# toposware/certificate-stark

Hardware: AMD Instinct MI355X
Metric: proofs/sec, state_transition AIR @ 2^20 steps (complete prove(): trace gen, LDE, Blake3 commitments, constraint evaluation, composition, DEEP, FRI, 96 queries) (higher is better)
Workload: dtype u64 (63-bit prime field, Montgomery) + u32 (Blake3)

## Files before the change

certificate-stark_amd/csrc/capi.hip:

```cpp
#include <hip/hip_runtime.h>
#include <stdio.h>
#include <stdlib.h>
#include <string.h>
#include <deque>
#include <new>
#include <vector>
#include "../../include/cstark.h"
#include "air_tx_host.h"
#include "blake3.h"
#include "ctx.h"
#include "constraints.h"
#include "deep.h"
#include "ext.h"
#include "hostfield.h"
#include "ntt.h"
#include "trace_gen.h"

namespace cs { thread_local char g_err[512] = ""; }
using cs::fail;
using cs::NttPlan;
using cs::CosetTable;
using cs::PeriodicTable;
using cs::g_err;

namespace {

struct DevGuard {
    std::vector<void *> ptrs;
    bool armed = true;
    template <class T> hipError_t alloc(T **p, size_t bytes) {
        const hipError_t e = hipMalloc((void **)p, bytes);
        if (e == hipSuccess) ptrs.push_back(*p);
        return e;
    }
    void release() { armed = false; }
    ~DevGuard() { if (armed) for (void *q : ptrs) (void)hipFree(q); }
};

int get_plan(cstark_ctx *c, unsigned log_n, const NttPlan **out) {
    for (const NttPlan &p : c->plans)
        if (p.log_n == log_n) { *out = &p; return CSTARK_OK; }
    const size_t n = (size_t)1 << log_n;
    NttPlan p{log_n, nullptr, nullptr, 0};
    DevGuard g;
    HIP_TRY(g.alloc(&p.w, n * 8));
    HIP_TRY(g.alloc(&p.winv, n * 8));
    const uint64_t w = cs::host::root_of_unity(log_n);
    HIP_TRY(cs::ntt_power_table(p.w, n, w, c->stream));
    HIP_TRY(cs::ntt_power_table(p.winv, n, cs::host::inv(w), c->stream));
    p.n_inv = cs::host::inv(cs::host::from_u64(n));
    cs::NttThreeStepShape shape;
    if (cs::ntt_three_step_shape(log_n, &shape)) {
        const size_t words = cs::ntt_aux_plan_words(shape);
        HIP_TRY(g.alloc(&p.aux_w, words * 8));
        HIP_TRY(g.alloc(&p.aux_winv, words * 8));
        HIP_TRY(cs::ntt_build_aux_plan(p.aux_w, p.w, shape, c->stream));
        HIP_TRY(cs::ntt_build_aux_plan(p.aux_winv, p.winv, shape, c->stream));
    }
    c->plans.push_back(p);
    g.release();
    *out = &c->plans.back();
    return CSTARK_OK;
}

int get_coset_table(cstark_ctx *c, unsigned log_n, unsigned log_b, uint64_t offset, const CosetTable **out) {
    for (const CosetTable &t : c->cosets)
        if (t.log_n == log_n && t.log_b == log_b && t.offset == offset) { *out = &t; return CSTARK_OK; }
    const size_t n = (size_t)1 << log_n, b = (size_t)1 << log_b;
    CosetTable t{log_n, log_b, offset, nullptr};
    DevGuard g;
    HIP_TRY(g.alloc(&t.s, b * n * 8));
    const uint64_t wbn = cs::host::root_of_unity(log_n + log_b);
    uint64_t shift = offset;
    for (size_t k = 0; k < b; k++) {
        HIP_TRY(cs::ntt_power_table(t.s + k * n, n, shift, c->stream));
        shift = cs::host::mul(shift, wbn);
    }
    cs::NttThreeStepShape shape;
    if (cs::ntt_three_step_shape(log_n, &shape)) {
        const NttPlan *p;
        RC_TRY(get_plan(c, log_n, &p));
        t.aux_words = cs::ntt_aux_coset_words(shape);
        HIP_TRY(g.alloc(&t.aux, b * t.aux_words * 8));
        for (size_t k = 0; k < b; k++) HIP_TRY(cs::ntt_build_aux_coset(t.aux + k * t.aux_words, p->w, t.s + k * n, shape, c->stream));
    }
    c->cosets.push_back(t);
    g.release();
    *out = &c->cosets.back();
    return CSTARK_OK;
}

int ensure_ws(cstark_ctx *c, size_t bytes) {
    if (bytes <= c->ws_bytes) return CSTARK_OK;
    if (c->ws) { HIP_TRY(hipStreamSynchronize(c->stream)); HIP_TRY(hipFree(c->ws)); c->ws = nullptr; c->ws_bytes = 0; }
    HIP_TRY(hipMalloc(&c->ws, bytes));
    c->ws_bytes = bytes;
// ... 181 lines not shown
int get_periodic(cstark_ctx *c, unsigned depth, unsigned log_n, unsigned log_b, const PeriodicTable **out) {
    for (const PeriodicTable &t : c->periodic)
        if (t.depth == depth && t.log_n == log_n && t.log_b == log_b) { *out = &t; return CSTARK_OK; }
    if (log_n < 10) return fail(CSTARK_ERR_INVALID_ARG, "the trace must hold at least one 1024-row transaction");
    std::vector<uint64_t> cols;
    if (!cs::host::tx_periodic_columns(depth, cols)) return fail(CSTARK_ERR_INVALID_ARG, "unsupported Merkle depth");
    static_assert(cs::host::TX_CYCLE == 1 << 10, "the cycle of TransactionAir's periodic columns");
    const size_t n = (size_t)1 << log_n, b = (size_t)1 << log_b;
    PeriodicTable t{depth, log_n, log_b, nullptr, nullptr, nullptr};
    DevGuard keep;
    RC_TRY(extend_periodic_columns(c, cols, cs::host::TX_NUM_PERIODIC, 10, log_n, log_b, keep, &t.tab));
    HIP_TRY(keep.alloc(&t.coset, b * cs::CE_COSET_CONSTS * 8));
    const uint64_t g = cs::host::lde_offset();
    std::vector<uint64_t> cc(b * cs::CE_COSET_CONSTS);
    const uint64_t wbn = cs::host::root_of_unity(log_n + log_b);
    uint64_t shift = g;
    for (size_t k = 0; k < b; k++) {
        uint64_t *o = cc.data() + k * cs::CE_COSET_CONSTS;
        o[0] = shift;
        o[1] = cs::host::inv(cs::host::sub(cs::host::pow(shift, n), cs::host::ONE));
        for (int gi = 0; gi < 5; gi++) o[2 + gi] = cs::host::pow(shift, cs::host::tx_group_adjustment(gi, n, n * b));
        o[7] = cs::host::pow(shift, cs::host::tx_boundary_adjustment(n, n * b));
        o[8] = cs::host::pow(shift, n - 1);
        o[9] = 0;
        shift = cs::host::mul(shift, wbn);
    }
    HIP_TRY(hipMemcpyAsync(t.coset, cc.data(), cc.size() * 8, hipMemcpyHostToDevice, c->stream));
    const NttPlan *plan;
    RC_TRY(get_plan(c, log_n, &plan));
    HIP_TRY(keep.alloc(&t.binv, b * 2 * n * 8));
    HIP_TRY(cs::build_boundary_inverses(t.binv, plan->w, t.coset, cs::host::inv(cs::host::root_of_unity(log_n)), log_n, log_b, c->stream));
    HIP_TRY(hipStreamSynchronize(c->stream));
    keep.release();
    c->periodic.push_back(t);
    *out = &c->periodic.back();
    return CSTARK_OK;
}

int get_small_periodic(cstark_ctx *c, int air, unsigned depth, unsigned log_n, unsigned log_b, const PeriodicTable **out) {
    for (const PeriodicTable &t : c->small_periodic)
        if (t.air == air && t.depth == depth && t.log_n == log_n && t.log_b == log_b) { *out = &t; return CSTARK_OK; }
    PeriodicTable t{depth, log_n, log_b, nullptr, nullptr, nullptr, air};
    std::vector<uint64_t> cols;
    DevGuard keep;
    if (air == CSTARK_AIR_MERKLE_UPDATE) {
        if (!cs::host::merkle_periodic_columns(depth, cols)) return fail(CSTARK_ERR_INVALID_ARG, "unsupported Merkle depth");
        RC_TRY(extend_periodic_columns(c, cols, 33, 9, log_n, log_b, keep, &t.tab));
    } else if (air == CSTARK_AIR_SCHNORR) {
        cs::host::schnorr_mask_columns(cols);
        RC_TRY(extend_periodic_columns(c, cols, 36, 9, log_n, log_b, keep, &t.tab));
    } else if (air == CSTARK_AIR_RESCUE_CHAIN) {
        using namespace cs::host;
        rescue_chain_periodic_columns(cols);
        const size_t n = (size_t)1 << log_n, b = (size_t)1 << log_b;
        for (int cidx = 0; cidx < 29; cidx++) intt_small(cols.data() + (size_t)cidx * 8, 3);
        std::vector<uint64_t> tab(b * 29 * 8);
        const uint64_t wbn = root_of_unity(log_n + log_b), w8 = root_of_unity(3);
        uint64_t shift = lde_offset();
        for (size_t k = 0; k < b; k++) {
            uint64_t x = pow(shift, n / 8);
            for (int m = 0; m < 8; m++) {
                for (int cidx = 0; cidx < 29; cidx++) {
                    const uint64_t *co = cols.data() + (size_t)cidx * 8;
                    uint64_t v = 0;
                    for (int d = 7; d >= 0; d--) v = add(mul(v, x), co[d]);
                    tab[(k * 29 + cidx) * 8 + m] = v;
                }
                x = mul(x, w8);
            }
            shift = mul(shift, wbn);
        }
        HIP_TRY(keep.alloc(&t.tab, tab.size() * 8));
        HIP_TRY(hipMemcpyAsync(t.tab, tab.data(), tab.size() * 8, hipMemcpyHostToDevice, c->stream));
        HIP_TRY(hipStreamSynchronize(c->stream));
    } else {
        return fail(CSTARK_ERR_UNSUPPORTED, "AIR not available through the generic entry points");
    }
    keep.release();
    c->small_periodic.push_back(t);
    *out = &c->small_periodic.back();
    return CSTARK_OK;
}

int ce_params(cstark_ctx *c, const uint64_t *d_lde, uint64_t *d_out, uint32_t merkle_depth, uint32_t log_n, uint32_t log_blowup, uint32_t k0,
              uint32_t nk, cs::CeParams *p) {
    if (!c || !d_lde || !d_out) return fail(CSTARK_ERR_INVALID_ARG, "constraint evaluation: null argument");
    if (((uintptr_t)d_lde & 15) != 0) return fail(CSTARK_ERR_INVALID_ARG, "constraint evaluation: d_lde must be 16-byte aligned (16-byte LDS-DMA pieces)");
    if (log_n < 10 || log_n > cs::NTT_MAX_LOG_N) return fail(CSTARK_ERR_INVALID_ARG, "trace length must be 2^10 .. 2^24");
    if (log_blowup != 3) return fail(CSTARK_ERR_UNSUPPORTED, "TransactionAir needs a constraint-evaluation blowup of 8 (max degree 7, src/air.rs:76-108)");
    if ((uint64_t)k0 + nk > (1ull << log_blowup) || nk == 0) return fail(CSTARK_ERR_INVALID_ARG, "coset range exceeds the blowup factor");
    HIP_TRY(hipSetDevice(c->device));
    const PeriodicTable *pt;
    const NttPlan *plan;
    RC_TRY(get_periodic(c, merkle_depth, log_n, log_blowup, &pt));
    RC_TRY(get_plan(c, log_n, &plan));
    const uint64_t n = 1ull << log_n, ce = n << log_blowup;
    *p = cs::CeParams{};
    p->lde = d_lde; p->ptab = pt->tab; p->w = plan->w; p->coset = pt->coset; p->binv = pt->binv; p->out = d_out;
    p->w_last = cs::host::inv(cs::host::root_of_unity(log_n));
    for (int g = 0; g < 5; g++) p->adj_mod_n[g] = (uint32_t)(cs::host::tx_group_adjustment(g, n, ce) & (n - 1));
    p->badj_mod_n = (uint32_t)(cs::host::tx_boundary_adjustment(n, ce) & (n - 1));
    p->log_n = log_n; p->log_b = log_blowup; p->k0 = k0;
    return CSTARK_OK;
}

}

int tx_witness_reserve(cstark_ctx *c, size_t n, size_t d, size_t *sz, size_t *off) {
    cs::witness_segments(n, d, sz, off);
    const size_t total = off[cs::WIT_NUM_SEGMENTS];
    if (total > c->wit_bytes) {
        if (c->wit_buf) { HIP_TRY(hipStreamSynchronize(c->stream)); HIP_TRY(hipFree(c->wit_buf)); c->wit_buf = nullptr; c->wit_bytes = 0; }
        HIP_TRY(hipMalloc(&c->wit_buf, total));
        c->wit_bytes = total;
    }
    return CSTARK_OK;
}
void tx_witness_bind(cstark_ctx *c, size_t n, size_t d, const size_t *off) {
    char *base = (char *)c->wit_buf;
    cs::TxWitnessDev &dv = c->wit;
    dv.n_tx = (uint32_t)n;
    dv.depth = (uint32_t)d;
    dv.initial_roots = (const uint64_t *)(base + off[cs::WIT_INITIAL_ROOTS]);
    dv.s_old = (const uint64_t *)(base + off[cs::WIT_S_OLD]);
    dv.r_old = (const uint64_t *)(base + off[cs::WIT_R_OLD]);
    dv.s_idx = (const uint64_t *)(base + off[cs::WIT_S_IDX]);
    dv.r_idx = (const uint64_t *)(base + off[cs::WIT_R_IDX]);
    dv.s_paths = (const uint64_t *)(base + off[cs::WIT_S_PATHS]);
    dv.r_paths = (const uint64_t *)(base + off[cs::WIT_R_PATHS]);
    dv.deltas = (const uint64_t *)(base + off[cs::WIT_DELTAS]);
    dv.sig_rx = (const uint64_t *)(base + off[cs::WIT_SIG_RX]);
    dv.h_limbs = (uint64_t *)(base + off[cs::WIT_H_LIMBS]);
    dv.sig_s = (const uint8_t *)(base + off[cs::WIT_SIG_S]);
    dv.msg_tail = nullptr;
}

extern "C" {

const char *cstark_last_error(void) { return g_err; }
const char *cstark_version(void) { return "certificate-stark_amd 0.2 (gfx950)"; }

int cstark_ctx_create(int device, void *stream, cstark_ctx **out) {
    if (!out) return fail(CSTARK_ERR_INVALID_ARG, "cstark_ctx_create: out is null");
    int count = 0;
    if (hipGetDeviceCount(&count) != hipSuccess || count == 0)
        return fail(CSTARK_ERR_NO_DEVICE, "no HIP device visible (this backend has no CPU fallback)");
    if (device < 0) HIP_TRY(hipGetDevice(&device));
    if (device >= count) return fail(CSTARK_ERR_INVALID_ARG, "device index out of range");
    HIP_TRY(hipSetDevice(device));
    cstark_ctx *c = new (std::nothrow) cstark_ctx();
    if (!c) return fail(CSTARK_ERR_OOM, "host allocation failed");
    c->device = device;
    c->stream = (hipStream_t)stream;
    int prio_lo = 0, prio_hi = 0;
    (void)hipDeviceGetStreamPriorityRange(&prio_lo, &prio_hi);
    if (hipStreamCreateWithPriority(&c->side, hipStreamNonBlocking, prio_hi) != hipSuccess ||
        hipStreamCreateWithPriority(&c->side2, hipStreamNonBlocking, prio_hi) != hipSuccess ||
        hipEventCreateWithFlags(&c->ev_fork, hipEventDisableTiming) != hipSuccess || hipEventCreateWithFlags(&c->ev_join, hipEventDisableTiming) != hipSuccess ||
        hipEventCreateWithFlags(&c->ev_join2, hipEventDisableTiming) != hipSuccess || hipEventCreateWithFlags(&c->ev_mid, hipEventDisableTiming) != hipSuccess) {
        delete c;
        return fail(CSTARK_ERR_HIP, "could not create the internal stream / events");
    }
    *out = c;
    return CSTARK_OK;
}
int cstark_ctx_create_own_stream(int device, cstark_ctx **out) {
    if (!out) return fail(CSTARK_ERR_INVALID_ARG, "cstark_ctx_create_own_stream: out is null");
    RC_TRY(cstark_ctx_create(device, nullptr, out));
    cstark_ctx *c = *out;
    if (hipStreamCreateWithFlags(&c->stream, hipStreamNonBlocking) != hipSuccess) {
        c->stream = nullptr;
        cstark_ctx_destroy(c);
        *out = nullptr;
        return fail(CSTARK_ERR_HIP, "could not create the context's stream");
    }
    c->owns_stream = true;
    return CSTARK_OK;
}

void cstark_ctx_destroy(cstark_ctx *c) {
    if (!c) return;
    (void)hipSetDevice(c->device);
    (void)hipStreamSynchronize(c->stream);
    if (c->side) { (void)hipStreamSynchronize(c->side); (void)hipStreamDestroy(c->side); }
    if (c->side2) { (void)hipStreamSynchronize(c->side2); (void)hipStreamDestroy(c->side2); }
    if (c->ev_join2) (void)hipEventDestroy(c->ev_join2);
    if (c->ev_mid) (void)hipEventDestroy(c->ev_mid);
    if (c->ev_fork) (void)hipEventDestroy(c->ev_fork);
    if (c->ev_join) (void)hipEventDestroy(c->ev_join);
    if (c->wit_buf) (void)hipFree(c->wit_buf);
    if (c->ws) (void)hipFree(c->ws);
    if (c->coef_buf) (void)hipFree(c->coef_buf);
    if (c->coef_stage) (void)hipHostFree(c->coef_stage);
    if (c->coef_ev) (void)hipEventDestroy(c->coef_ev);
    for (NttPlan &p : c->plans) { (void)hipFree(p.w); (void)hipFree(p.winv); (void)hipFree(p.aux_w); (void)hipFree(p.aux_winv); }
    for (CosetTable &t : c->cosets) { (void)hipFree(t.s); (void)hipFree(t.aux); }
    for (cs::StepTable &t : c->steps) { (void)hipFree(t.d); (void)hipFree(t.w); }
    for (PeriodicTable &t : c->periodic) { (void)hipFree(t.tab); (void)hipFree(t.coset); (void)hipFree(t.binv); }
    for (PeriodicTable &t : c->small_periodic) (void)hipFree(t.tab);
    for (cs::AssertInverseTable &t : c->assert_inv) (void)hipFree(t.tab);
    for (cs::AirCombineStatic &t : c->air_static) (void)hipFree(t.d_static);
    if (c->air_coef_buf) (void)hipFree(c->air_coef_buf);
    if (c->air_coef_stage) (void)hipHostFree(c->air_coef_stage);
    if (c->air_coef_ev) (void)hipEventDestroy(c->air_coef_ev);
    if (c->deep_buf) (void)hipFree(c->deep_buf);
    if (c->deep_stage) (void)hipHostFree(c->deep_stage);
    if (c->deep_ev) (void)hipEventDestroy(c->deep_ev);
    if (c->desc_buf) (void)hipFree(c->desc_buf);
    if (c->rb_dev) (void)hipFree(c->rb_dev);
    if (c->shard_bit37) (void)hipFree(c->shard_bit37);
    if (c->rb_host) (void)hipHostFree(c->rb_host);
    if (c->tail_buf) (void)hipFree(c->tail_buf);
    if (c->arena) cs::prove_arena_free(c->arena);
    if (c->verify) cs::verify_arena_free(c->verify);
    for (hipEvent_t e : c->part_ev) if (e) (void)hipEventDestroy(e);
    for (hipEvent_t e : c->lde_ev) (void)hipEventDestroy(e);
    if (c->owns_stream && c->stream) (void)hipStreamDestroy(c->stream);
    delete c;
}

int cstark_ctx_synchronize(cstark_ctx *c) {
    if (!c) return fail(CSTARK_ERR_INVALID_ARG, "null context");
    HIP_TRY(hipStreamSynchronize(c->stream));
    return CSTARK_OK;
}

int cstark_malloc(cstark_ctx *c, size_t bytes, void **d_ptr) {
    if (!c || !d_ptr) return fail(CSTARK_ERR_INVALID_ARG, "cstark_malloc: null argument");
    HIP_TRY(hipSetDevice(c->device));
    HIP_TRY(hipMalloc(d_ptr, bytes));
    return CSTARK_OK;
}
int cstark_free(cstark_ctx *c, void *d_ptr) {
    if (!c) return fail(CSTARK_ERR_INVALID_ARG, "null context");
    HIP_TRY(hipSetDevice(c->device));
    HIP_TRY(hipStreamSynchronize(c->stream));
    HIP_TRY(hipFree(d_ptr));
    return CSTARK_OK;
}
int cstark_memcpy_h2d(cstark_ctx *c, void *d_dst, const void *src, size_t bytes) {
    if (!c || (!d_dst && bytes) || (!src && bytes)) return fail(CSTARK_ERR_INVALID_ARG, "cstark_memcpy_h2d: null argument");
    HIP_TRY(hipMemcpyAsync(d_dst, src, bytes, hipMemcpyHostToDevice, c->stream));
    HIP_TRY(hipStreamSynchronize(c->stream));
    return CSTARK_OK;
}
int cstark_memcpy_d2h(cstark_ctx *c, void *dst, const void *d_src, size_t bytes) {
    if (!c || (!dst && bytes) || (!d_src && bytes)) return fail(CSTARK_ERR_INVALID_ARG, "cstark_memcpy_d2h: null argument");
    HIP_TRY(hipMemcpyAsync(dst, d_src, bytes, hipMemcpyDeviceToHost, c->stream));
    HIP_TRY(hipStreamSynchronize(c->stream));
    return CSTARK_OK;
}

int cstark_tx_witness_upload(cstark_ctx *c, const cstark_tx_witness *w) {
    if (!c || !w) return fail(CSTARK_ERR_INVALID_ARG, "cstark_tx_witness_upload: null argument");
    const size_t n = w->n_tx, d = w->merkle_depth;
    if (n == 0) return fail(CSTARK_ERR_INVALID_ARG, "n_tx must be positive");
    if (d == 0 || ((d + 1) & d) != 0 || 8 * d + 7 > 511) return fail(CSTARK_ERR_INVALID_ARG, "tree depth must be one less than a power of 2 and at most 31");
    if (!w->initial_roots || !w->s_old_values || !w->r_old_values || !w->s_indices || !w->r_indices || !w->s_paths || !w->r_paths ||
        !w->deltas || !w->sig_rx || !w->sig_s)
        return fail(CSTARK_ERR_INVALID_ARG, "witness array pointer is null");
    HIP_TRY(hipSetDevice(c->device));
    const void *src[] = {w->initial_roots, w->s_old_values, w->r_old_values, w->s_indices, w->r_indices, w->s_paths, w->r_paths, w->deltas, w->sig_rx, nullptr, w->sig_s};
    size_t sz[cs::WIT_NUM_SEGMENTS], off[cs::WIT_NUM_SEGMENTS + 1];
    RC_TRY(tx_witness_reserve(c, n, d, sz, off));
    char *base = (char *)c->wit_buf;
    for (int i = 0; i < cs::WIT_NUM_SEGMENTS; i++)
        if (src[i]) HIP_TRY(hipMemcpyAsync(base + off[i], src[i], sz[i], hipMemcpyHostToDevice, c->stream));
    HIP_TRY(hipStreamSynchronize(c->stream));
    tx_witness_bind(c, n, d, off);
    return CSTARK_OK;
}

int cstark_tx_build_trace(cstark_ctx *c, uint64_t *d_trace) {
    if (!c || !d_trace) return fail(CSTARK_ERR_INVALID_ARG, "cstark_tx_build_trace: null argument");
    if (!c->wit_buf || c->wit.n_tx == 0) return fail(CSTARK_ERR_INVALID_ARG, "no witness uploaded");
// ... 465 lines not shown
    sm.desc.families = cs::CE_SPLIT_FAMILIES;
    sm.desc.tables_per_set = cs::CE_SPLIT_TABLES;
    sm.desc.raw_family = cs::CE_SPLIT_FAMILIES - 1;
    for (int f = 0; f < cs::CE_SPLIT_FAMILIES; f++) {
        sm.desc.terms[f] = count[f];
        for (int t = 0; t < count[f]; t++) sm.desc.term[f][t] = cs::coset_merge_term(first[f] + t, t ? adj[t - 1] : 0, log_n, g);
    }
    sm.hi = cs::coset_merge_term(0, adj[0], log_n, cs::host::mul(g, cs::host::root_of_unity(log_n + 3)), 2);
    sm.log_n = log_n;
    return sm;
}

namespace {

struct SplitStage {
    unsigned log_n;
    size_t n;
    const NttPlan *pn, *p4, *p8;
    const CosetTable *t1;
    hipStream_t stream;
};
int split_stage(cstark_ctx *c, unsigned log_n, SplitStage *s) {
    *s = SplitStage{log_n, (size_t)1 << log_n, nullptr, nullptr, nullptr, nullptr, c->stream};
    RC_TRY(get_plan(c, log_n, &s->pn));
    RC_TRY(get_plan(c, log_n + 2, &s->p4));
    RC_TRY(get_plan(c, log_n + 3, &s->p8));
    return get_coset_table(c, log_n, 3, cs::host::from_u64(1), &s->t1);
}

int inverse_columns(const SplitStage &s, const uint64_t *in, uint64_t *scratch, uint64_t *out, unsigned width, unsigned batch = 1, size_t batch_stride = 0) {
    cs::NttArgs a{};
    a.in = in; a.scratch = scratch; a.out = out; a.width = width; a.batch = batch; a.log_n = s.log_n;
    a.in_batch_stride = batch_stride; a.scratch_batch_stride = batch_stride; a.out_batch_stride = batch_stride;
    a.w = s.pn->winv; a.post_scale = s.pn->n_inv; a.do_scale = true; a.inverse = true; a.aux = s.pn->aux_winv;
    HIP_TRY(cs::ntt_columns(a, s.stream));
    return CSTARK_OK;
}

int forward_to_cosets(const SplitStage &s, unsigned first, const uint64_t *in, uint64_t *scratch, uint64_t *out, unsigned width, size_t in_batch_stride) {
    const CosetTable *t1 = s.t1;
    cs::NttArgs f{};
    f.in = in; f.scratch = scratch; f.out = out; f.width = width; f.batch = first == 1 ? 4 : 3; f.log_n = s.log_n;
    f.w = s.pn->w; f.prescale = t1->s + first * s.n; f.prescale_batch_stride = 2 * s.n; f.do_scale = false; f.inverse = false;
    f.aux = s.pn->aux_w; f.aux_ps = t1->aux ? t1->aux + first * t1->aux_words : nullptr; f.aux_ps_batch_stride = 2 * t1->aux_words;
    f.in_batch_stride = in_batch_stride; f.scratch_batch_stride = (size_t)width * s.n; f.out_batch_stride = (size_t)width * s.n;
    HIP_TRY(cs::ntt_columns(f, s.stream));
    return CSTARK_OK;
}

int even_to_odd(const SplitStage &s, const uint64_t *in, uint64_t *out, unsigned tables, unsigned kc0 = 0, unsigned nkc = 4) {
    HIP_TRY(cs::coset_even_to_odd(in, out, s.log_n, tables, s.p4->winv, s.p8->w, cs::host::inv(cs::host::from_u64(4)), s.stream, kc0, nkc));
    return CSTARK_OK;
}

struct SplitWs { uint64_t *even, *sa, *sb, *sc, *odd, *fin_direct, *fin_hi, *fin_co, *fin_scr, *fin_tco, *fin_hm; };
int split_ws_unmerged(cstark_ctx *c, size_t region, size_t hcol, SplitWs *w) {
    RC_TRY(ensure_ws(c, (5 * region + 9 * hcol) * 8));
    *w = SplitWs{};
    w->even = (uint64_t *)c->ws; w->sa = w->even + region; w->sb = w->sa + region; w->sc = w->sb + region; w->odd = w->sc + region;
    w->fin_direct = w->odd + region; w->fin_hi = w->fin_direct + hcol; w->fin_co = w->fin_hi + 4 * hcol; w->fin_scr = w->fin_co + hcol ;
    return CSTARK_OK;
}
int split_ws_merged(cstark_ctx *c, size_t region, size_t fregion, size_t hcol, SplitWs *w) {
    RC_TRY(ensure_ws(c, (3 * region + fregion + 8 * hcol) * 8));
    *w = SplitWs{};
    w->even = (uint64_t *)c->ws; w->sa = w->even + region; w->sb = w->sa + region; w->sc = w->sa + fregion; w->odd = w->sb + region;
    w->fin_direct = w->odd + fregion; w->fin_hi = w->fin_direct + hcol; w->fin_co = w->fin_hi + 2 * hcol; w->fin_tco = w->fin_co + hcol;
    w->fin_hm = w->fin_tco + hcol; w->fin_scr = w->fin_hm + 3 * hcol / 2;
    return CSTARK_OK;
}

int final_hi_unmerged(const SplitStage &s, const SplitWs &w, unsigned rows, unsigned first, unsigned per_set, unsigned tables_per_set) {
    HIP_TRY(cs::launch_final_hi(w.odd, w.fin_direct, w.fin_hi, cs::host::inv(cs::host::from_u64(2)), s.log_n, rows, first, per_set, tables_per_set, s.stream));
    RC_TRY(inverse_columns(s, w.fin_hi, w.fin_scr, w.fin_co, rows));
    return forward_to_cosets(s, 2, w.fin_co, w.fin_scr, w.fin_hi + (size_t)rows * s.n, rows, 0);
}

int tx_even_cosets(const cs::CeParams &p, uint64_t *even, size_t n, hipStream_t stream, hipEvent_t *pev) {
    if (pev) HIP_TRY(hipEventRecord(pev[0], stream));
    HIP_TRY(cs::launch_rounds_setup(p, stream));
    HIP_TRY(cs::launch_rounds_split(p, even, stream));
    if (pev) HIP_TRY(hipEventRecord(pev[1], stream));
    uint64_t *fam_dbl = even + (size_t)cs::CE_SPLIT_FAM0 * 4 * n, *fam_add = fam_dbl + 12 * n, *fam_addbit = fam_add + 8 * n;
    HIP_TRY(cs::launch_ec_split(p, 1, fam_dbl, nullptr, stream));
    if (pev) HIP_TRY(hipEventRecord(pev[2], stream));
    HIP_TRY(cs::launch_ec_split(p, 2, fam_add, nullptr, stream));
    if (pev) HIP_TRY(hipEventRecord(pev[3], stream));
    HIP_TRY(cs::launch_ec_split(p, 3, fam_dbl, nullptr, stream));
    if (pev) HIP_TRY(hipEventRecord(pev[4], stream));
    HIP_TRY(cs::launch_ec_split(p, 4, fam_addbit, fam_add, stream));
    if (pev) HIP_TRY(hipEventRecord(pev[5], stream));
    uint64_t *fam_final = fam_addbit + 8 * n;
    HIP_TRY(cs::launch_final_split(p, -1, fam_final, stream));
    if (pev) HIP_TRY(hipEventRecord(pev[6], stream));
    HIP_TRY(cs::launch_lin_all(p, even, stream));
    if (pev) { HIP_TRY(hipEventRecord(pev[7], stream)); HIP_TRY(hipEventRecord(pev[8], stream)); }
    return CSTARK_OK;
}

}

int tx_evaluate_constraints_sets(cstark_ctx *c, const uint64_t *d_lde, const cstark_tx_coeffs *coeffs, uint32_t m, const uint64_t pub_inputs[4],
                                 uint64_t *const *d_outs, uint32_t merkle_depth, uint32_t log_n, uint32_t log_blowup, uint32_t k0, uint32_t nk,
                                 bool input_is_lde, const uint64_t *d_pub) {
    if ((!pub_inputs && !d_pub) || !d_outs) return fail(CSTARK_ERR_INVALID_ARG, "cstark_tx_evaluate_constraints: null argument");
    if (m < 1 || m > (uint32_t)cs::CE_MAX_SETS) return fail(CSTARK_ERR_INVALID_ARG, "cstark_tx_evaluate_constraints: 1..3 coefficient sets");
    for (uint32_t q = 1; q < m; q++)
        if (!d_outs[q]) return fail(CSTARK_ERR_INVALID_ARG, "cstark_tx_evaluate_constraints: null output");
    cs::CeParams p;
    RC_TRY(ce_params(c, d_lde, d_outs[0], merkle_depth, log_n, log_blowup, k0, nk, &p));
    if (coeffs) RC_TRY(upload_coeffs(c, coeffs, m, p));
    else { RC_TRY(ensure_coef_buf(c)); p.coef = c->coef_buf; p.rtab = c->coef_buf + TX_COEF_WORDS; p.m = m; }
    for (uint32_t q = 1; q < m; q++) p.out_ext[q - 1] = d_outs[q];
    for (int i = 0; i < 4; i++) p.pub[i] = pub_inputs ? pub_inputs[i] : 0;
    p.pubd = d_pub;
    static const bool split_env = [] { const char *e = getenv("CSTARK_ROUNDS_SPLIT"); return !e || atoi(e) != 0; }();
    hipEvent_t *pev = c->part_timing ? c->part_ev : nullptr;
    if (split_env && input_is_lde && k0 == 0 && nk == 8 && log_n + 3 <= cs::NTT_MAX_LOG_N) {
        SplitStage st;
        RC_TRY(split_stage(c, log_n, &st));
        const size_t n = st.n;
        const unsigned T = cs::CE_SPLIT_TABLES * m;
        const size_t region = (size_t)T * 4 * n;
        const size_t hcol = (size_t)2 * m * n;
        static const bool split_merge_env = [] { const char *e = getenv("CSTARK_SPLIT_MERGE"); return !e || atoi(e) != 0; }();
        const unsigned F = cs::CE_SPLIT_FAMILIES * m;
        SplitWs w;
        if (split_merge_env) RC_TRY(split_ws_merged(c, region, (size_t)F * 4 * n, hcol, &w));
        else RC_TRY(split_ws_unmerged(c, region, hcol, &w));
        RC_TRY(tx_even_cosets(p, w.even, n, c->stream, pev));
        RC_TRY(inverse_columns(st, w.even, w.sa, w.sb, 4 * T));
        if (split_merge_env) {
            const SplitMerge &sm = tx_split_merge(log_n);
            HIP_TRY(cs::coset_even_to_odd_merged(w.sb, w.sa, log_n, m, sm.desc, st.p4->winv, st.p8->w, cs::host::inv(cs::host::from_u64(4)), w.fin_tco, c->stream));
            RC_TRY(forward_to_cosets(st, 1, w.sa, w.sc, w.odd, F, (size_t)F * n));
            const uint64_t half = cs::host::inv(cs::host::from_u64(2));
            HIP_TRY(cs::launch_final_split(p, 1, w.fin_direct, c->stream));
            HIP_TRY(cs::launch_final_hi_merged(p, w.odd, w.fin_direct, w.fin_hi, half, c->stream));
            RC_TRY(inverse_columns(st, w.fin_direct, w.fin_scr, w.fin_co, 2 * m));
            HIP_TRY(cs::launch_final_hi_merge(p, w.fin_tco, w.fin_co, w.fin_hm, sm.hi, half, c->stream));
            RC_TRY(forward_to_cosets(st, 2, w.fin_hm, w.fin_scr, w.fin_hi + (size_t)m * n, m, (size_t)m * n));
        } else {
            RC_TRY(even_to_odd(st, w.sb, w.sa, T));
            RC_TRY(forward_to_cosets(st, 1, w.sa, w.sc, w.odd, T, (size_t)T * n));
            HIP_TRY(cs::launch_final_split(p, 1, w.fin_direct, c->stream));
            RC_TRY(final_hi_unmerged(st, w, 2 * m, cs::CE_SPLIT_FINAL, 2, cs::CE_SPLIT_TABLES));
        }
        HIP_TRY(cs::launch_split_finish(p, w.even, w.odd, w.fin_hi, c->stream, split_merge_env));
        if (pev) HIP_TRY(hipEventRecord(pev[cs::CE_NUM_PARTS], c->stream));
    } else {
        HIP_TRY(cs::launch_eval_constraints(p, nk, c->stream, pev));
    }
    c->part_valid = c->part_timing;
    return CSTARK_OK;
}
int tx_evaluate_constraints_shard(cstark_ctx *c, const uint64_t *d_lde, const uint64_t *d_coeffs, const cstark_tx_coeffs *coeffs, const uint64_t pub_inputs[4],
                                  uint64_t *d_out, uint32_t merkle_depth, uint32_t log_n, uint32_t k0, uint32_t nk) {
    if (!coeffs || !pub_inputs || !d_out || !d_coeffs) return fail(CSTARK_ERR_INVALID_ARG, "sharded constraint evaluation: null argument");
    if ((nk != 2 && nk != 4) || (k0 % nk) || k0 + nk > 8) return fail(CSTARK_ERR_INVALID_ARG, "sharded split evaluation: a rank holds 2 or 4 consecutive cosets");
    if (log_n + 3 > cs::NTT_MAX_LOG_N) return fail(CSTARK_ERR_UNSUPPORTED, "trace too long for the split evaluation");
    cs::CeParams p;
    RC_TRY(ce_params(c, d_lde, d_out, merkle_depth, log_n, 3, k0, nk, &p));
    RC_TRY(upload_coeffs(c, coeffs, 1, p));
    for (int i = 0; i < 4; i++) p.pub[i] = pub_inputs[i];
    p.nkc = nk / 2;
    const unsigned kc0 = k0 / 2, nkc = nk / 2;
    SplitStage st;
    RC_TRY(split_stage(c, log_n, &st));
    const size_t n = st.n;
// ... 307 lines not shown
    p.w = plan->w;
    p.w_last = cs::host::inv(cs::host::root_of_unity(log_n));
    p.width = s.width; p.n_constraints = (uint32_t)nc; p.n_assertions = (uint32_t)na;
    p.stride = 1u << (log_b - s.log_ce_blowup()); p.log_n = log_n;
    static const bool inv_tables = [] { const char *e = getenv("CSTARK_AIR_INV_TABLES"); return !e || atoi(e) != 0; }();
    std::vector<cs::AssertInverseTable> built;
    for (uint32_t gi = 0; inv_tables && gi < p.n_agrp; gi++) {
        for (const cs::AssertInverseTable &t : c->assert_inv)
            if (t.log_n == log_n && t.log_b == log_b && t.m == p.agrp_m[gi] && t.zc == p.agrp_zc[gi]) p.agrp_inv[gi] = t.tab;
        if (p.agrp_inv[gi]) continue;
        cs::AssertInverseTable t{log_n, log_b, p.agrp_m[gi], p.agrp_zc[gi], nullptr};
        HIP_TRY(g.alloc(&t.tab, (size_t)b * (n / t.m) * 8));
        uint64_t sm[8] = {};
        for (uint64_t k = 0; k < b; k++) sm[k] = p.agrp_mshift[k][gi];
        HIP_TRY(cs::launch_assert_inverses(t.tab, plan->w, sm, (unsigned)b, t.m, t.zc, log_n, c->stream));
        p.agrp_inv[gi] = t.tab;
        built.push_back(t);
    }
    g.release();
    for (const cs::AssertInverseTable &t : built) c->assert_inv.push_back(t);
    c->air_static.push_back(std::move(q));
    *out = &c->air_static.back();
    return CSTARK_OK;
}

int stage_air_coefs(cstark_ctx *c, const AirStageRequest &rq, const cs::host::AirShape &s, const cs::AirCombineStatic &st, cs::AirCombineParams &p,
                    const uint64_t **d_txl, uint64_t **d_rtab) {
    constexpr size_t TXL = 230;
    const size_t nc = s.n_constraints, na = s.a_reg.size();
    const size_t words = 2 * nc + 3 * na + TXL, total = words + cs::MERKLE_RTAB_WORDS;
    if (c->air_coef_words < total) {
        if (rq.d_coefs && c->air_coef_words) HIP_TRY(hipEventSynchronize(c->air_coef_ev));
        HIP_TRY(hipStreamSynchronize(c->stream));
        if (c->air_coef_buf) { HIP_TRY(hipFree(c->air_coef_buf)); c->air_coef_buf = nullptr; }
        if (c->air_coef_stage) { HIP_TRY(hipHostFree(c->air_coef_stage)); c->air_coef_stage = nullptr; }
        c->air_coef_words = 0;
        HIP_TRY(hipMalloc((void **)&c->air_coef_buf, total * 8));
        HIP_TRY(hipHostMalloc((void **)&c->air_coef_stage, total * 8, hipHostMallocDefault));
        if (!c->air_coef_ev) HIP_TRY(hipEventCreateWithFlags(&c->air_coef_ev, hipEventDisableTiming));
        c->air_coef_words = total;
    } else if (!rq.d_coefs) {
        HIP_TRY(hipEventSynchronize(c->air_coef_ev));
    }
    const uint64_t *d = c->air_coef_buf;
    *d_rtab = c->air_coef_buf + words;
    if (rq.d_coefs) {
        p.t_alpha = rq.d_coefs; p.t_beta = rq.d_coefs + 115; p.b_alpha = rq.d_coefs + 230; p.b_beta = rq.d_coefs + 230 + na;
        p.a_value = rq.d_avalues ? rq.d_avalues : st.d_static + ((size_t)1 << rq.log_blowup);
        *d_txl = rq.d_coefs;
        return CSTARK_OK;
    }
    uint64_t *q = c->air_coef_stage;
    memcpy(q, rq.t_alpha, nc * 8); q += nc;
    memcpy(q, rq.t_beta, nc * 8); q += nc;
    memcpy(q, rq.b_alpha, na * 8); q += na;
    memcpy(q, rq.b_beta, na * 8); q += na;
    for (size_t a = 0; a < na; a++) *q++ = s.a_const.empty() ? rq.assertion_values[a] : s.a_const[a];
    memset(q, 0, TXL * 8);
    if (nc <= 115) { memcpy(q, rq.t_alpha, nc * 8); memcpy(q + 115, rq.t_beta, nc * 8); }
    HIP_TRY(hipMemcpyAsync(c->air_coef_buf, c->air_coef_stage, words * 8, hipMemcpyHostToDevice, c->stream));
    HIP_TRY(hipEventRecord(c->air_coef_ev, c->stream));
    p.t_alpha = d; p.t_beta = d + nc;
    p.b_alpha = d + 2 * nc; p.b_beta = d + 2 * nc + na; p.a_value = d + 2 * nc + 2 * na;
    *d_txl = d + 2 * nc + 3 * na;
    return CSTARK_OK;
}

int schnorr_transition_sum(cstark_ctx *c, const AirStageRequest &rq, const cs::AirCombineParams &p, const std::vector<uint32_t> &t_grp, const uint64_t *d_txl,
                           uint64_t *d_rtab) {
    const PeriodicTable *pt;
    RC_TRY(get_small_periodic(c, CSTARK_AIR_SCHNORR, 0, rq.log_n, rq.log_blowup, &pt));
    static const bool split_env = [] { const char *e = getenv("CSTARK_SCHNORR_SPLIT"); return !e || atoi(e) != 0; }();
    if (!(split_env && rq.own_extension && rq.k0 == 0 && rq.nk == 8 && rq.log_blowup == 3 && rq.log_n >= 12 && rq.log_n + 3 <= cs::NTT_MAX_LOG_N && rq.n_items > 1)) {
        HIP_TRY(cs::launch_schnorr_fused(p, rq.d_aux_lde, pt->tab, rq.nk, c->stream));
        return CSTARK_OK;
    }
    static const bool final5 = [] { const char *e = getenv("CSTARK_SCHNORR_FINAL5"); return !e || atoi(e) != 0; }();
    const unsigned T = final5 ? cs::SCHNORR_SPLIT_TABLES : cs::SCHNORR_SPLIT_EC_TABLES;
    SplitStage st;
    RC_TRY(split_stage(c, rq.log_n, &st));
    const size_t n = st.n, region = (size_t)T * 4 * n, hcol = (size_t)3 * n;
    SplitWs w;
    RC_TRY(split_ws_unmerged(c, region, hcol, &w));
    HIP_TRY(cs::launch_schnorr_ec_split(p, rq.d_aux_lde, d_txl, w.even, c->stream));
    if (final5) HIP_TRY(cs::launch_schnorr_final_split(p, d_txl, w.even + (size_t)cs::SCHNORR_SPLIT_EC_TABLES * 4 * n, -1, c->stream));
    RC_TRY(inverse_columns(st, w.even, w.sa, w.sb, 4 * T));
    RC_TRY(even_to_odd(st, w.sb, w.sa, T));
    RC_TRY(forward_to_cosets(st, 1, w.sa, w.sc, w.odd, T, (size_t)T * n));
    if (final5) {
        HIP_TRY(cs::launch_schnorr_final_split(p, d_txl, w.fin_direct, 1, c->stream));
        RC_TRY(final_hi_unmerged(st, w, 3, cs::SCHNORR_SPLIT_EC_TABLES, 3, cs::SCHNORR_SPLIT_TABLES));
    }
    static const bool rounds_env = [] { const char *e = getenv("CSTARK_SCHNORR_ROUNDS"); return !e || atoi(e) != 0; }();
    HIP_TRY(cs::launch_schnorr_split_finish(p, rq.d_aux_lde, pt->tab, w.even, w.odd, t_grp[0], t_grp[6], c->stream, rounds_env ? d_rtab : nullptr, t_grp[42],
                                            final5 ? w.fin_hi : nullptr));
    return CSTARK_OK;
}

int merkle_transition_sum(cstark_ctx *c, const AirStageRequest &rq, const cs::AirCombineParams &p, const std::vector<uint32_t> &t_grp, uint64_t *d_rtab) {
    const PeriodicTable *pt;
    RC_TRY(get_small_periodic(c, CSTARK_AIR_MERKLE_UPDATE, rq.merkle_depth, rq.log_n, rq.log_blowup, &pt));
    static const bool rounds_env = [] { const char *e = getenv("CSTARK_MERKLE_ROUNDS"); return !e || atoi(e) != 0; }();
    HIP_TRY(cs::launch_merkle_fused(p, pt->tab, rq.nk, c->stream, rounds_env ? d_rtab : nullptr, t_grp[0]));
    return CSTARK_OK;
}

}

int air_stage(cstark_ctx *c, const AirStageRequest &rq) {
    cs::host::AirShape s;
    RC_TRY(air_stage_validate(c, rq, s));
    HIP_TRY(hipSetDevice(c->device));
    const cs::AirCombineStatic *st;
    RC_TRY(get_air_static(c, rq, s, &st));
    cs::AirCombineParams p = st->p;
    p.lde = rq.d_lde; p.evals = rq.d_evals; p.out = rq.d_out; p.avals = rq.d_avals_lde; p.n_avals = rq.n_avals; p.k0 = rq.k0;
    const uint64_t *d_txl;
    uint64_t *d_rtab;
    RC_TRY(stage_air_coefs(c, rq, s, *st, p, &d_txl, &d_rtab));
    if (rq.source == AirTransitions::SchnorrFused) RC_TRY(schnorr_transition_sum(c, rq, p, st->t_grp, d_txl, d_rtab));
    if (rq.source == AirTransitions::MerkleFused) RC_TRY(merkle_transition_sum(c, rq, p, st->t_grp, d_rtab));
    if (rq.source != AirTransitions::Materialised) p.tsum = rq.d_out;
    HIP_TRY(cs::launch_air_combine(p, rq.nk, c->stream));
    return CSTARK_OK;
}

extern "C" {

int cstark_air_combine(cstark_ctx *c, int air, uint32_t n_items, const uint64_t *d_lde, const uint64_t *d_evals, const uint64_t *t_alpha,
                       const uint64_t *t_beta, const uint64_t *b_alpha, const uint64_t *b_beta, const uint64_t *assertion_values,
                       const uint64_t *d_avals_lde, uint32_t n_avals, uint64_t *d_out, uint32_t log_n, uint32_t log_blowup, uint32_t k0, uint32_t nk) {
    if (!d_evals) return fail(CSTARK_ERR_INVALID_ARG, "cstark_air_combine: null argument");
    AirStageRequest rq;
    rq.air = air; rq.n_items = n_items;
    rq.log_n = log_n; rq.log_blowup = log_blowup; rq.k0 = k0; rq.nk = nk;
    rq.d_lde = d_lde; rq.d_out = d_out;
    rq.source = AirTransitions::Materialised; rq.d_evals = d_evals;
    rq.t_alpha = t_alpha; rq.t_beta = t_beta; rq.b_alpha = b_alpha; rq.b_beta = b_beta; rq.assertion_values = assertion_values;
    rq.d_avals_lde = d_avals_lde; rq.n_avals = n_avals;
    return air_stage(c, rq);
}
int cstark_merkle_evaluate_constraints(cstark_ctx *c, uint32_t merkle_depth, const uint64_t *d_lde, const uint64_t *t_alpha, const uint64_t *t_beta,
                                       const uint64_t *b_alpha, const uint64_t *b_beta, const uint64_t *assertion_values, uint64_t *d_out, uint32_t log_n,
                                       uint32_t log_blowup, uint32_t k0, uint32_t nk) {
    if (merkle_depth > 31) return fail(CSTARK_ERR_INVALID_ARG, "cstark_merkle_evaluate_constraints: unsupported Merkle depth");
    AirStageRequest rq;
    rq.air = CSTARK_AIR_MERKLE_UPDATE;
    rq.log_n = log_n; rq.log_blowup = log_blowup; rq.k0 = k0; rq.nk = nk;
    rq.d_lde = d_lde; rq.d_out = d_out;
    rq.source = AirTransitions::MerkleFused; rq.merkle_depth = merkle_depth;
    rq.t_alpha = t_alpha; rq.t_beta = t_beta; rq.b_alpha = b_alpha; rq.b_beta = b_beta; rq.assertion_values = assertion_values;
    return air_stage(c, rq);
}
int cstark_schnorr_evaluate_constraints(cstark_ctx *c, uint32_t n_sig, const uint64_t *d_lde, const uint64_t *d_aux_lde, const uint64_t *t_alpha,
                                        const uint64_t *t_beta, const uint64_t *b_alpha, const uint64_t *b_beta, const uint64_t *d_avals_lde,
                                        uint32_t n_avals, uint64_t *d_out, uint32_t log_n, uint32_t log_blowup, uint32_t k0, uint32_t nk) {
    if (!d_aux_lde) return fail(CSTARK_ERR_INVALID_ARG, "cstark_schnorr_evaluate_constraints: null argument");
    AirStageRequest rq;
    rq.air = CSTARK_AIR_SCHNORR; rq.n_items = n_sig;
    rq.log_n = log_n; rq.log_blowup = log_blowup; rq.k0 = k0; rq.nk = nk;
    rq.d_lde = d_lde; rq.d_out = d_out;
    rq.source = AirTransitions::SchnorrFused; rq.d_aux_lde = d_aux_lde;
    rq.t_alpha = t_alpha; rq.t_beta = t_beta; rq.b_alpha = b_alpha; rq.b_beta = b_beta;
    rq.d_avals_lde = d_avals_lde; rq.n_avals = n_avals;
    return air_stage(c, rq);
}
int cstark_schnorr_evaluate_constraints_lde(cstark_ctx *c, uint32_t n_sig, const uint64_t *d_lde, const uint64_t *d_aux_lde, const uint64_t *t_alpha,
// ... 61 lines not shown
```

certificate-stark_amd/csrc/constraints.h:

```cpp
#pragma once
#include <hip/hip_runtime.h>
#include <stddef.h>
#include <stdint.h>
#include "ntt.h"

namespace cs {

__host__ __device__ constexpr int tx_degree_group(int i) {
    return (i < 6 || (i >= 19 && i < 37)) ? 0 : (i >= 6 && i < 18) ? 1 : (i == 18 || (i >= 37 && i < 58)) ? 2 : (i == 92) ? 3 : 4;
}
constexpr unsigned TX_GROUP_BASE[5] = {5, 4, 3, 2, 1};
constexpr unsigned TX_GROUP_CYCLES[5] = {2, 2, 1, 1, 1};

constexpr int CE_RTAB_WORDS = 12288;
constexpr int CE_COEF_WORDS = 115 * 2 + 8;
constexpr int CE_MAX_SETS = 3;
constexpr int CE_COSET_CONSTS = 10;

struct CeParams {
    const uint64_t *lde;
    const uint64_t *ptab;
    const uint64_t *w;
    const uint64_t *coset;
    const uint64_t *coef;
    const uint64_t *binv;
    uint64_t *rtab;
    uint64_t *out;
    uint64_t *out_ext[CE_MAX_SETS - 1];
    uint32_t m;
    uint64_t pub[4];
    const uint64_t *pubd;
    uint64_t w_last;
    uint32_t adj_mod_n[5];
    uint32_t badj_mod_n;
    uint32_t log_n, log_b, k0;
    uint32_t nkc;
};

constexpr int AIR_MAX_GROUPS = 8;
struct AirCombineParams {
    const uint64_t *lde, *evals, *w, *shifts;
    const uint64_t *t_alpha, *t_beta;
    const uint64_t *b_alpha, *b_beta, *a_value;
    const uint32_t *a_reg;
    const int32_t *a_seq;
    const uint64_t *avals;
    const uint64_t *tsum;
    uint64_t *out;
    uint64_t w_last;
    uint32_t width, n_constraints, n_assertions, n_avals, stride, log_n, k0;
    const uint32_t *t_grp, *a_grp;
    uint32_t n_tgrp, n_agrp;
    uint64_t tgrp_adj[AIR_MAX_GROUPS], agrp_m[AIR_MAX_GROUPS], agrp_zc[AIR_MAX_GROUPS], agrp_badj[AIR_MAX_GROUPS];
    uint64_t tgrp_shift[8][AIR_MAX_GROUPS], agrp_bshift[8][AIR_MAX_GROUPS], agrp_mshift[8][AIR_MAX_GROUPS], zinv_coset[8];
    const uint64_t *agrp_inv[AIR_MAX_GROUPS];
};
hipError_t launch_assert_inverses(uint64_t *d_tab, const uint64_t *d_w, const uint64_t shift_m[8], unsigned b, uint64_t m, uint64_t zc, unsigned log_n,
                                  hipStream_t stream);
hipError_t launch_air_combine(const AirCombineParams &p, unsigned nk, hipStream_t stream);
hipError_t launch_eval_transitions_merkle(const uint64_t *lde, const uint64_t *ptab, uint64_t *out, unsigned log_n, unsigned k0, unsigned nk,
                                          hipStream_t stream);
hipError_t launch_eval_transitions_schnorr(const uint64_t *lde, const uint64_t *aux, const uint64_t *ptab, uint64_t *out, unsigned log_n, unsigned k0,
                                           unsigned nk, hipStream_t stream);
constexpr int MERKLE_RTAB_WORDS = 2048;
hipError_t launch_merkle_fused(const AirCombineParams &p, const uint64_t *ptab, unsigned nk, hipStream_t stream, uint64_t *d_rtab = nullptr,
                               unsigned round_group = 0);
hipError_t launch_schnorr_fused(const AirCombineParams &p, const uint64_t *aux, const uint64_t *ptab, unsigned nk, hipStream_t stream);
constexpr int SCHNORR_SPLIT_EC_TABLES = 8, SCHNORR_SPLIT_TABLES = 11;
hipError_t launch_schnorr_ec_split(const AirCombineParams &p, const uint64_t *aux, const uint64_t *d_coefs_tx_layout, uint64_t *d_even, hipStream_t stream);
hipError_t launch_schnorr_split_finish(const AirCombineParams &p, const uint64_t *aux, const uint64_t *ptab, const uint64_t *d_even, const uint64_t *d_odd,
                                       unsigned g0, unsigned g1, hipStream_t stream, uint64_t *d_rtab = nullptr, unsigned round_group = 0,
                                       const uint64_t *d_hi = nullptr);
hipError_t launch_schnorr_final_split(const AirCombineParams &p, const uint64_t *d_coefs_tx_layout, uint64_t *d_out, int coset, hipStream_t stream);
hipError_t launch_eval_transitions_range(const uint64_t *lde, uint64_t *out, unsigned log_n, unsigned nk, hipStream_t stream);
hipError_t launch_eval_transitions_rescue(const uint64_t *lde, const uint64_t *ptab, uint64_t *out, unsigned log_n, unsigned k0, unsigned nk,
                                          hipStream_t stream);

hipError_t launch_eval_transitions(const CeParams &p, unsigned nk, hipStream_t stream);
hipError_t launch_eval_frames(const uint64_t *cur, const uint64_t *next, const uint64_t *per, uint64_t *out, unsigned nf, hipStream_t stream);
hipError_t launch_eval_frames_air(int air, const uint64_t *cur, const uint64_t *next, const uint64_t *per, uint64_t *out, unsigned nf, hipStream_t stream);
constexpr int CE_NUM_PARTS = 9;
hipError_t launch_eval_constraints(const CeParams &p, unsigned nk, hipStream_t stream, hipEvent_t *part_events = nullptr);
hipError_t launch_rounds_setup(const CeParams &p, hipStream_t stream);
hipError_t launch_rounds_split(const CeParams &p, uint64_t *d_even, hipStream_t stream);
hipError_t launch_ec_split(const CeParams &p, int part, uint64_t *d_even_family, uint64_t *d_even_linear, hipStream_t stream);
constexpr int CE_SPLIT_TABLES = 13, CE_SPLIT_FAM0 = 4, CE_SPLIT_FINAL = 11;
hipError_t launch_lin_all(const CeParams &p, uint64_t *d_even_family0, hipStream_t stream);
hipError_t launch_split_finish_shard(const CeParams &p, const uint64_t *d_even, const uint64_t *d_odd, const uint64_t *d_hi, const uint64_t *d_bit37_all,
                                     uint64_t *d_out, hipStream_t stream);
hipError_t launch_shard_combine(const uint64_t *d_parts, uint64_t *d_out, unsigned log_n, unsigned nkc, hipStream_t stream);
constexpr int CE_SPLIT_FAMILIES = 5;
hipError_t launch_split_finish(const CeParams &p, const uint64_t *d_even, const uint64_t *d_odd, const uint64_t *d_hi, hipStream_t stream,
                               bool merged = false);
hipError_t launch_final_split(const CeParams &p, int coset, uint64_t *d_out, hipStream_t stream);
hipError_t launch_final_hi(const uint64_t *d_odd, const uint64_t *d_direct, uint64_t *d_hi, uint64_t half , unsigned log_n,
                           unsigned rows, unsigned first, unsigned per_set, unsigned tables_per_set, hipStream_t stream);
hipError_t launch_final_hi_merged(const CeParams &p, const uint64_t *d_odd, const uint64_t *d_direct, uint64_t *d_hi, uint64_t half, hipStream_t stream);
hipError_t launch_final_hi_merge(const CeParams &p, const uint64_t *d_tco, const uint64_t *d_qco, uint64_t *d_out, const CosetMergeTerm &tm, uint64_t half,
                                 hipStream_t stream);
hipError_t build_boundary_inverses(uint64_t *d_table, const uint64_t *d_w, const uint64_t *d_coset, uint64_t w_last, unsigned log_n, unsigned log_b,
                                   hipStream_t stream);

}
```

certificate-stark_amd/csrc/constraints.hip:

```cpp
#include <type_traits>
#include "constraints.h"
#include "mds_mfma.cuh"
#include "rounds_layout.h"
#include "rescue.cuh"
#include "tower.cuh"

namespace cs {
namespace {

constexpr int NT = 128;

enum {
    S_INIT = 0, S_UPD = 15, R_INIT = 29, R_UPD = 44, PREV_ROOT = 58, S_KEY = 65, R_KEY = 77, DELTA_COPY = 89, SIGMA_COPY = 90,
    NONCE_COPY = 91, DELTA_BIT = 56, DELTA_ACC = 57, SIGMA_BIT = 92, SIGMA_ACC = 93,
    VALUE_RES = 65, BALANCE_RES = 90, NONCE_UPD_RES = 91, INT_ROOT_RES = 92, PREV_MATCH_RES = 99, S_KEY_RES = 101, R_KEY_RES = 103,
    DELTA_COPY_RES = 105, SIGMA_COPY_RES = 106, NONCE_COPY_RES = 107, DELTA_RANGE_RES = 108, SIGMA_RANGE_RES = 109,
    P_SETUP = 0, P_MERKLE = 1, P_HASH_INPUT = 2, P_FINISH = 3, P_HASH = 4, P_SCHNORR = 5, P_SCALAR_MULT = 6, P_DOUBLING = 7,
    P_DIGEST = 8, P_SCHNORR_HASH = 12, P_HASH_INTERNAL = 13, P_RANGE_STEP = 17, P_RANGE_FINISH = 18, P_VALUE_COPY = 19, P_ARK = 20
};

struct Frame {
    const fp *cur_p, *next_p, *per_p;
    size_t n;
    unsigned pcycle;
// ... 332 lines not shown
#define CS_ROUNDS_UNROLL 1
#endif
constexpr int ROUNDS_UNROLL = CS_ROUNDS_UNROLL;
enum { PART_ROUNDS = 0, PART_DBL0, PART_ADD0, PART_DBL1, PART_ADD1, PART_FINAL, PART_LIN_A, PART_LIN_B, PART_LIN_C, NUM_PARTS };

#define CS_CONST __attribute__((address_space(4)))
template <class T>
__device__ __forceinline__ const CS_CONST T *as_const(const T *p) { return (const CS_CONST T *)(uintptr_t)p; }

template <int M>
struct Fused {
    const CS_CONST fp *coefs;
    const fp *xp;
    Acc128 s[M];
    int cnt;
    fp total[M];
    __device__ __forceinline__ fp coef(int c, int i) const {
        const CS_CONST fp *a = coefs + c * CE_COEF_WORDS;
        return fp_add(a[i], fp_mul(a[115 + i], xp[tx_degree_group(i) * FNT + threadIdx.x]));
    }
    __device__ __forceinline__ void begin() {
#pragma unroll
        for (int c = 0; c < M; c++) s[c] = acc_zero();
        cnt = 0;
    }
    __device__ __forceinline__ void term(int i, fp v) {
        ++cnt;
#pragma unroll
        for (int c = 0; c < M; c++) {
            acc_mad(s[c], coef(c, i), v);
            if (cnt == 7) acc_fold(s[c]);
        }
        if (cnt == 7) cnt = 0;
    }
    __device__ __forceinline__ void end(fp flag) {
#pragma unroll
        for (int c = 0; c < M; c++) {
            acc_fold(s[c]);
            total[c] = fp_add(total[c], fp_mul(flag, acc_reduce(s[c])));
        }
    }
    __device__ __forceinline__ void add(int c, fp v) { total[c] = fp_add(total[c], v); }
};

__device__ __forceinline__ fp dot14(const fp *__restrict__ m, const fp (&x)[14]) {
    Acc128 a = acc_zero();
#pragma unroll
    for (int j = 0; j < 7; j++) acc_mad(a, m[j], x[j]);
    acc_fold(a);
#pragma unroll
    for (int j = 7; j < 14; j++) acc_mad(a, m[j], x[j]);
    acc_fold(a);
    return acc_reduce(a);
}

__device__ __forceinline__ fp dot14l(const CS_CONST uint32_t *m, const fp (&x)[14]) {
    uint64_t c00 = 0, c01 = 0, c02 = 0, c10 = 0, c11 = 0, c12 = 0;
#pragma unroll
    for (int j = 0; j < 14; j++) {
        const uint32_t x0 = (uint32_t)x[j], x1 = (uint32_t)(x[j] >> 32);
        const uint32_t m0 = m[4 * j], m1 = m[4 * j + 1], m2 = m[4 * j + 2];
        c00 = mad_u64_u32(x0, m0, c00); c01 = mad_u64_u32(x0, m1, c01); c02 = mad_u64_u32(x0, m2, c02);
        c10 = mad_u64_u32(x1, m0, c10); c11 = mad_u64_u32(x1, m1, c11); c12 = mad_u64_u32(x1, m2, c12);
    }
    typedef unsigned __int128 u128;
    const u128 v = ((u128)c00 + ((u128)c10 << 32)) + (((u128)c01 + ((u128)c11 << 32)) << 21) + (((u128)c02 + ((u128)c12 << 32)) << 42);
    Acc128 a{(uint64_t)v, (uint64_t)(v >> 64)};
    acc_fold(a);
    return acc_reduce(a);
}
__device__ __forceinline__ void split_limbs(fp v, uint32_t *out4) {
    out4[0] = (uint32_t)v & 0x1fffffu; out4[1] = (uint32_t)(v >> 21) & 0x1fffffu; out4[2] = (uint32_t)(v >> 42); out4[3] = 0;
}

__constant__ RoundWindow c_windows[5] = CS_ROUND_WINDOWS_INIT;
__constant__ int c_window_groups[5][2][3] = CS_WINDOW_GROUPS_INIT;
constexpr size_t ROUNDS_LDS = MT_BYTES + (FNT / 64) * 64 * mdsmfma::ROW_BYTES;
#ifdef CS_ROUNDS_MFMA
constexpr size_t ROUNDS_DYN_LDS = ROUNDS_LDS;
#else
constexpr size_t ROUNDS_DYN_LDS = 0;
#endif

__global__ void k_rounds_setup(const fp *__restrict__ coef, const fp *__restrict__ ptab, fp *__restrict__ rtab) {
    coef += (size_t)blockIdx.y * CE_COEF_WORDS;
    rtab += (size_t)blockIdx.y * CE_RTAB_WORDS;
    if (blockIdx.x >= RT_SECTIONS) {
        if (threadIdx.x < 16) mdsmfma::build_table_entry((uint8_t *)(rtab + RT_MT), c_inv_mds, 14, blockIdx.x - RT_SECTIONS, threadIdx.x);
        return;
    }
    const int sec = blockIdx.x, wdx = sec >> 3, fs = (sec >> 2) & 1, slot = sec & 3;
    const RoundWindow w = c_windows[wdx];
    const int res = fs ? w.res_b : w.res_a;
    const int grp = slot ? c_window_groups[wdx][fs][slot - 1] : -2;
    const bool used = (fs == 0 || w.flag_b >= 0) && grp != -1;
    __shared__ fp gam[14];
    if (threadIdx.x < 14) {
        const int i = res + threadIdx.x;
        gam[threadIdx.x] = !used ? 0 : slot == 0 ? coef[i] : (tx_degree_group(i) == grp ? coef[115 + i] : 0);
    }
    __syncthreads();
    const int t = threadIdx.x;
    if (t < 14) rtab[RT_G + sec * 14 + t] = gam[t];
    if (t < 14) {
        fp u = 0;
        for (int i = 0; i < 14; i++) u = fp_add(u, fp_mul(gam[i], c_mds[i * 14 + t]));
        split_limbs(u, (uint32_t *)(rtab + RT_UL) + (sec * 14 + t) * 4);
    }
    if (sec == 0)
        for (int e = t; e < 196; e += blockDim.x) split_limbs(c_inv_mds[e], (uint32_t *)(rtab + RT_ML) + e * 4);
    if (t < 64) {
        const int k = t >> 3, r = t & 7;
        fp a = 0;
        for (int i = 0; i < 14; i++) a = fp_add(a, fp_mul(gam[i], ptab[((size_t)k * 48 + P_ARK + i) * 1024 + r]));
        rtab[RT_A + sec * 64 + t] = a;
    }
}

constexpr int RW_ROWS = 66, RW_IMG = 14 * RW_ROWS;
typedef __attribute__((address_space(3))) void lds_void;
typedef const __attribute__((address_space(1))) void glb_void;
__device__ __forceinline__ void rounds_fetch_window(const fp *rows, size_t n, int reg, int lane, fp *img) {
    if (lane < 33) {
#pragma unroll
        for (int j = 0; j < 14; j++)
            __builtin_amdgcn_global_load_lds((glb_void *)(rows + (size_t)(reg + j) * n), (lds_void *)(img + j * RW_ROWS), 16, 0, 0);
    }
}
template <int M>
__device__ __forceinline__ void fused_rounds(Fused<M> &acc, const Frame &f, const fp *__restrict__ rtab, unsigned k, unsigned jr, const uint8_t *mtab,
                                             uint8_t *stage, const fp *ark2_lds, const fp *atab_lds, fp *img, const fp *colbase) {
    const int lane = threadIdx.x & 63;
    const fp *ark2 = ark2_lds + jr * 14;
    const fp flags[4] = {f.pv(P_SETUP), f.pv(P_HASH), f.pv(P_SCHNORR_HASH), fp_add(f.pv(P_SETUP), f.pv(P_HASH))};
    const fp *atab = atab_lds + jr;
    const CS_CONST uint32_t *ul = as_const((const uint32_t *)(rtab + RT_UL));
    const fp *rows = f.cur_p + lane;
    if (lane == 32 && ((size_t)(f.cur_p - lane + 64 - colbase) & (f.n - 1)) == 0) rows -= f.n;
    rounds_fetch_window(rows, f.n, c_windows[0].reg, lane, img);
#pragma unroll 1
    for (int wdx = 0; wdx < 5; wdx++) {
        const RoundWindow w = c_windows[wdx];
        asm volatile("s_waitcnt vmcnt(0)" ::: "memory");
        fp d[14];
#pragma unroll
        for (int j = 0; j < 14; j++) d[j] = fp_sub(img[j * RW_ROWS + lane + 1], ark2[j]);
#ifdef CS_ROUNDS_MFMA
        fp yv[14];
        {
            mdsmfma::stage_vector(stage, lane, d);
            __builtin_amdgcn_wave_barrier();
            mdsmfma::BFrags bf;
            mdsmfma::load_bfrags(bf, stage, lane);
            __builtin_amdgcn_wave_barrier();
            uint64_t *img = (uint64_t *)stage;
            constexpr int RW = mdsmfma::ROW_BYTES / 8;
#pragma unroll
            for (int T = 0; T < 7; T++) {
                fp y2[2];
                mdsmfma::tile_product(mtab, 7, T, bf, lane, y2);
                img[(lane & 31) * RW + 2 * T + (lane >> 5)] = y2[0];
                img[(32 + (lane & 31)) * RW + 2 * T + (lane >> 5)] = y2[1];
            }
            __builtin_amdgcn_wave_barrier();
#pragma unroll
            for (int i = 0; i < 14; i++) yv[i] = img[lane * RW + i];
            __builtin_amdgcn_wave_barrier();
        }
#endif
// ... 322 lines not shown
__device__ __forceinline__ void fused_doubling(A &acc, const Frame &f, int reg, fp doubling) {
    const Point p = {load6(f, reg, false), load6(f, reg + 6, false), load6(f, reg + 12, false)};
    const Point d = ec_double<CS_EC_CALL>(p);
    acc.begin();
#pragma unroll
    for (int i = 0; i < 6; i++) {
        acc.term(reg + i, fp_sub(f.next(reg + i), d.x.c[i]));
        acc.term(reg + 6 + i, fp_sub(f.next(reg + 6 + i), d.y.c[i]));
        acc.term(reg + 12 + i, fp_sub(f.next(reg + 12 + i), d.z.c[i]));
    }
    acc.term(reg + 18, c_is_binary(f.cur(reg + 18)));
    acc.end(doubling);
}
template <class A>
__device__ __forceinline__ void fused_addition(A &acc, const Frame &f, int reg, const Fp6 &qx, const Fp6 &qy, fp addition) {
    const Point p = {load6(f, reg, false), load6(f, reg + 6, false), load6(f, reg + 12, false)};
    const fp bit = f.cur(reg + 18);
    const Point a = ec_add_mixed<CS_EC_CALL>(p, qx, qy);
    acc.begin();
#pragma unroll
    for (int i = 0; i < 6; i++) {
        acc.term(reg + i, fp_sub(fp_sub(f.next(reg + i), f.cur(reg + i)), fp_mul(bit, fp_sub(a.x.c[i], f.cur(reg + i)))));
        acc.term(reg + 6 + i, fp_sub(fp_sub(f.next(reg + 6 + i), f.cur(reg + 6 + i)), fp_mul(bit, fp_sub(a.y.c[i], f.cur(reg + 6 + i)))));
        acc.term(reg + 12 + i, fp_sub(fp_sub(f.next(reg + 12 + i), f.cur(reg + 12 + i)), fp_mul(bit, fp_sub(a.z.c[i], f.cur(reg + 12 + i)))));
    }
    acc.term(reg + 18, fp_sub(bit, f.next(reg + 18)));
    acc.end(addition);
}
template <class A>
__device__ __forceinline__ void fused_final_addition(A &acc, const Frame &f, fp final_add) {
    const Point sp = {load6(f, 0, false), load6(f, 6, false), load6(f, 12, false)};
    const Point hp = {load6(f, 19, false), load6(f, 25, false), load6(f, 31, false)};
    const Point r = ec_add<CS_EC_CALL>(sp, hp);
    const Fp6 xz = mul6(load6(f, 0, true), r.z);
    acc.begin();
#pragma unroll
    for (int i = 0; i < 6; i++) {
        acc.term(i, fp_sub(xz.c[i], r.x.c[i]));
        acc.term(6 + i, fp_sub(f.next(6 + i), r.y.c[i]));
        acc.term(12 + i, fp_sub(f.next(12 + i), r.z.c[i]));
    }
    acc.end(final_add);
}

template <int M>
struct SplitAcc {
    const CS_CONST fp *coefs;
    Acc128 sa[M], sb[M][2];
    int ca, cb[2];
    __device__ __forceinline__ void begin() {
        ca = cb[0] = cb[1] = 0;
#pragma unroll
        for (int c = 0; c < M; c++) sa[c] = sb[c][0] = sb[c][1] = acc_zero();
    }
    __device__ __forceinline__ void term(int i, fp v) {
        if (i == 18 || i == 37) return;
        const bool fa = ++ca == 7;
#pragma unroll
        for (int c = 0; c < M; c++) {
            acc_mad(sa[c], coefs[c * CE_COEF_WORDS + i], v);
            if (fa) acc_fold(sa[c]);
        }
        if (fa) ca = 0;
        const int g = tx_degree_group(i);
#pragma unroll
        for (int q = 0; q < 2; q++)
            if (g == q) {
                const bool fb = ++cb[q] == 7;
#pragma unroll
                for (int c = 0; c < M; c++) {
                    acc_mad(sb[c][q], coefs[c * CE_COEF_WORDS + 115 + i], v);
                    if (fb) acc_fold(sb[c][q]);
                }
                if (fb) cb[q] = 0;
            }
    }
    __device__ __forceinline__ void end(fp) {}
    __device__ __forceinline__ fp result(int c, int q) {
        Acc128 &a = q == 0 ? sa[c] : sb[c][q == 0 ? 0 : q - 1];
        acc_fold(a);
        return acc_reduce(a);
    }
};
template <int PART, bool ACCUMULATE, int M>
#ifndef CS_EC_WAVES
#define CS_EC_WAVES 2
#endif
__global__ __launch_bounds__(FNT, CS_EC_WAVES) void k_ec_split(CeParams p, fp *__restrict__ out, fp *__restrict__ out_linear) {
    const size_t n = (size_t)1 << p.log_n;
    const size_t j = blockIdx.x * (size_t)FNT + threadIdx.x;
    const unsigned kc = (p.k0 >> 1) + blockIdx.y;
    const Frame f = make_frame(p, 2 * blockIdx.y, j);
    SplitAcc<M> acc;
    acc.coefs = as_const(p.coef);
    constexpr size_t SET = (size_t)SPLIT_TABLES * 4;
    if (PART == PART_DBL0) fused_doubling(acc, f, 0, (fp)0);
    if (PART == PART_DBL1) fused_doubling(acc, f, 19, (fp)0);
    if (PART == PART_ADD0) fused_addition(acc, f, 0, const6(c_generator), const6(c_generator + 6), (fp)0);
    if (PART == PART_ADD1) {
        acc.begin();
#pragma unroll
        for (int i = 0; i < 18; i++) acc.term(19 + i, fp_sub(f.next(19 + i), f.cur(19 + i)));
#pragma unroll
        for (int c = 0; c < M; c++)
#pragma unroll
            for (int q = 0; q < 2; q++) {
                fp *o = out_linear + (c * SET + (size_t)q * 4 + kc) * n + j;
                *o = fp_add(*o, acc.result(c, q));
            }
        const Point pt = {load6(f, 19, false), load6(f, 25, false), load6(f, 31, false)};
        const Point a = ec_add_mixed<CS_EC_CALL>(pt, load6(f, S_KEY, true), load6(f, S_KEY + 6, true));
        acc.begin();
#pragma unroll
        for (int i = 0; i < 6; i++) {
            acc.term(19 + i, fp_sub(a.x.c[i], pt.x.c[i]));
            acc.term(25 + i, fp_sub(a.y.c[i], pt.y.c[i]));
            acc.term(31 + i, fp_sub(a.z.c[i], pt.z.c[i]));
        }
    }
    constexpr int NQ = (PART == PART_ADD1 || PART == PART_ADD0) ? 2 : 3;
    const fp xd1 = PART == PART_ADD0 ? split_lift(p, 2 * kc, j) : 0;
#pragma unroll
    for (int c = 0; c < M; c++)
#pragma unroll
        for (int q = 0; q < NQ; q++) {
            fp *o = out + (c * SET + (size_t)q * 4 + kc) * n + j;
            fp v = acc.result(c, q);
            if (PART == PART_ADD0 && q == 1) v = fp_add(v, fp_mul(xd1, acc.result(c, 2)));
            *o = ACCUMULATE ? fp_add(*o, v) : v;
        }
}

template <int M>
__global__ __launch_bounds__(FNT, CS_EC_WAVES) void k_final_split(CeParams p, fp *__restrict__ out, int coset) {
    const size_t n = (size_t)1 << p.log_n;
    const size_t j = blockIdx.x * (size_t)FNT + threadIdx.x;
    const unsigned kc = (p.k0 >> 1) + blockIdx.y, k = coset < 0 ? 2 * kc : (unsigned)coset;
    const Frame f = make_frame(p, k - p.k0, j);
    SplitAcc<M> acc;
    acc.coefs = as_const(p.coef);
    fused_final_addition(acc, f, (fp)0);
    const fp xd1 = split_lift(p, k, j);
    constexpr size_t SET = (size_t)SPLIT_TABLES * 4;
#pragma unroll
    for (int c = 0; c < M; c++) {
        const fp a = acc.result(c, 0), b = fp_add(acc.result(c, 1), fp_mul(xd1, acc.result(c, 2)));
        if (coset < 0) {
            out[(c * SET + kc) * n + j] = a;
            out[(c * SET + 4 + kc) * n + j] = b;
        } else {
            out[((size_t)c * 2) * n + j] = a;
            out[((size_t)c * 2 + 1) * n + j] = b;
        }
    }
}
__global__ __launch_bounds__(256) void k_final_hi(const fp *__restrict__ odd, const fp *__restrict__ direct, fp *__restrict__ hi, fp half, unsigned log_n,
                                                  unsigned first, unsigned per_set, unsigned tables_per_set) {
    const size_t n = (size_t)1 << log_n;
    const size_t j = blockIdx.x * (size_t)256 + threadIdx.x;
    const unsigned r = blockIdx.y;
    const fp t = odd[((size_t)(r / per_set) * tables_per_set + first + r % per_set) * n + j];
    hi[(size_t)r * n + j] = fp_mul(fp_sub(t, direct[(size_t)r * n + j]), half);
}

template <int M>
__global__ __launch_bounds__(256) void k_final_hi_merged(CeParams p, const fp *__restrict__ odd, const fp *__restrict__ direct, fp *__restrict__ hi, fp half) {
    const size_t n = (size_t)1 << p.log_n;
    const size_t j = blockIdx.x * (size_t)256 + threadIdx.x;
    const unsigned c = blockIdx.y;
    const fp xp0 = fp_mul(p.coset[CE_COSET_CONSTS + 2], p.w[(j * p.adj_mod_n[0]) & (n - 1)]);
    const fp q = fp_add(direct[((size_t)c * 2) * n + j], fp_mul(direct[((size_t)c * 2 + 1) * n + j], xp0));
    hi[(size_t)c * n + j] = fp_mul(fp_sub(odd[((size_t)c * SPLIT_FAMILIES + SPLIT_FAMILIES - 1) * n + j], q), half);
}
template <int M>
__global__ __launch_bounds__(256) void k_final_hi_merge(const fp *__restrict__ tco, const fp *__restrict__ qco, fp *__restrict__ out, size_t n,
                                                        CosetMergeTerm tm, fp half) {
    const size_t q = blockIdx.x * (size_t)256 + threadIdx.x;
    const unsigned c = blockIdx.y;
    const size_t qs = (q - tm.r) & (n - 1);
    const size_t i0 = ((size_t)c * 2) * n + q, i1 = ((size_t)c * 2 + 1) * n + qs;
    const fp h0 = fp_mul(fp_sub(tco[i0], qco[i0]), half), h1 = fp_mul(fp_sub(tco[i1], qco[i1]), half);
#pragma unroll
    for (int i = 0; i < 3; i++) out[((size_t)i * M + c) * n + q] = fp_add(h0, fp_mul(h1, tm.c[i][q < tm.r ? 1 : 0]));
}

template <int M, class A>
__device__ __forceinline__ void fused_merkle_auth_rest_sets(A &acc, const Frame &f, int base, fp tx_hash, fp hash_copy, fp hash_init) {
    const fp bit = f.next(base + 14), not_bit = c_not(bit);
    acc.begin();
    acc.term(base + 14, c_is_binary(bit));
    acc.end(tx_hash);
    Acc128 s_copy[M], s_init[M];
#pragma unroll
    for (int c = 0; c < M; c++) s_copy[c] = s_init[c] = acc_zero();
#pragma unroll 1
    for (int i = 0; i < 7; i++) {
        const fp ca = f.cur(base + i), na0 = f.next(base + i), cb = f.cur(base + 15 + i), nb0 = f.next(base + 15 + i);
        const fp na7 = f.next(base + 7 + i), nb7 = f.next(base + 22 + i);
        const fp da = fp_sub(ca, na0), db = fp_sub(cb, nb0);
        const fp u0 = fp_add(fp_mul(not_bit, da), fp_mul(bit, fp_sub(nb0, na0)));
        const fp u7 = fp_add(fp_mul(bit, fp_sub(ca, na7)), fp_mul(not_bit, fp_sub(nb7, na7)));
        const fp u15 = fp_mul(not_bit, db), u22 = fp_mul(bit, fp_sub(cb, nb7));
#pragma unroll
        for (int c = 0; c < M; c++) {
            const fp c0 = acc.coef(c, base + i), c15 = acc.coef(c, base + 15 + i);
            acc_mad(s_copy[c], c0, da);
            acc_mad(s_copy[c], c15, db);
            acc_mad(s_init[c], c0, u0);
            acc_mad(s_init[c], acc.coef(c, base + 7 + i), u7);
            acc_mad(s_init[c], c15, u15);
            acc_mad(s_init[c], acc.coef(c, base + 22 + i), u22);
// ... 641 lines not shown
    if constexpr (PART == 0) {
#pragma unroll 1
        for (int i = 0; i < 56; i++) out[(size_t)i * nf + j] = 0;
    }
    AccAll acc{out + j, nf};
    schnorr_transitions<PART>(acc, f, fr, per + (size_t)36 * nf + j, nf);
}
struct AirSum {
    const CS_CONST fp *alpha, *beta;
    const CS_CONST uint32_t *grp;
    const fp *xp;
    Acc128 s;
    int cnt;
    fp total;
    __device__ __forceinline__ fp coef(int i) const { return fp_add(alpha[i], fp_mul(beta[i], xp[grp[i] * FNT + threadIdx.x])); }
    __device__ __forceinline__ void begin() { s = acc_zero(); cnt = 0; }
    __device__ __forceinline__ void term(int i, fp v) {
        acc_mad(s, coef(i), v);
        if (++cnt == 7) { acc_fold(s); cnt = 0; }
    }
    __device__ __forceinline__ void end(fp flag) {
        acc_fold(s);
        total = fp_add(total, fp_mul(flag, acc_reduce(s)));
    }
    __device__ __forceinline__ void add(int i, fp flag, fp val) { total = fp_add(total, fp_mul(coef(i), fp_mul(flag, val))); }
};
enum { SF_DBL0 = 0, SF_ADD0, SF_DBL1, SF_ADD1, SF_FINAL, SF_REST, SF_PARTS };
template <int PART, bool AFTER_SPLIT = false, bool FOLDED_ROUND = false>
__global__ __launch_bounds__(FNT, PART == SF_REST ? 2 : CS_EC_WAVES) void k_schnorr_fused(AirCombineParams p, const fp *__restrict__ aux,
                                                                                       const fp *__restrict__ ptab) {
    __shared__ fp xp_lds[AIR_MAX_GROUPS * FNT];
    const size_t n = (size_t)1 << p.log_n;
    const size_t j = blockIdx.x * (size_t)FNT + threadIdx.x;
    const unsigned kk = blockIdx.y, k = p.k0 + kk;
    const fp *base = p.lde + (size_t)kk * 56 * n;
    Frame f;
    f.n = n;
    f.cur_p = base + j;
    f.next_p = base + ((j + 1) & (n - 1));
    f.per_p = ptab + (size_t)k * 36 * 512 + (j & 511);
    f.pcycle = 512;
    for (unsigned g = 0; g < p.n_tgrp; g++) xp_lds[g * FNT + threadIdx.x] = fp_mul(p.tgrp_shift[k][g], p.w[(j * p.tgrp_adj[g]) & (n - 1)]);
    AirSum acc{as_const(p.t_alpha), as_const(p.t_beta), as_const(p.t_grp), xp_lds, acc_zero(), 0, 0};
    const fp *ax = aux + (size_t)kk * 19 * n + j;
    const fp global_mask = f.pv(0), scalar_mult = f.pv(1), doubling = f.pv(2), hash_flag = f.pv(7);
    const fp addition = fp_mul(c_not(doubling), scalar_mult);
    if constexpr (PART == SF_DBL0) fused_doubling(acc, f, 0, doubling);
    if constexpr (PART == SF_DBL1) fused_doubling(acc, f, 19, doubling);
    if constexpr (PART == SF_ADD0) fused_addition(acc, f, 0, const6(c_generator), const6(c_generator + 6), addition);
    if constexpr (PART == SF_ADD1) fused_addition(acc, f, 19, fp6_load_strided(ax, n), fp6_load_strided(ax + 6 * n, n), addition);
    if constexpr (PART == SF_FINAL) fused_final_addition(acc, f, fp_mul(c_not(scalar_mult), global_mask));
    if constexpr (PART == SF_REST) {
        const fp copy_hash = fp_mul(c_not(hash_flag), global_mask), final_add = fp_mul(c_not(scalar_mult), global_mask);
        Frame fr = f;
        fr.per_p = f.per_p - (size_t)(P_ARK - 8) * 512;
#pragma unroll 1
        for (int i = 0; i < 4; i++) {
            const fp dflag = f.pv(3 + i);
            const fp c = f.cur(41 - i), nx = f.next(41 - i);
            acc.add(41 - i, fp_mul(dflag, doubling), fp_sub(nx, fp_add(fp_dbl(c), f.next(37))));
            acc.add(41 - i, fp_mul(c_not(dflag), doubling), fp_sub(c, nx));
            acc.add(38 + i, addition, fp_sub(f.cur(38 + i), f.next(38 + i)));
            acc.add(38 + i, final_add, fp_sub(f.cur(38 + i), f.cur(42 + i)));
        }
        if (!FOLDED_ROUND) enforce_round(acc, fr, 42, 42, hash_flag, 0, 0, false);
#pragma unroll 1
        for (int i = 0; i < 7; i++) {
            acc.add(42 + i, copy_hash, fp_sub(f.cur(42 + i), f.next(42 + i)));
            acc.add(49 + i, copy_hash, fp_sub(f.next(49 + i), ax[(size_t)(12 + i) * n]));
        }
        if (AFTER_SPLIT) {
            const fp b18 = f.cur(18), b37 = f.cur(37);
            acc.add(18, doubling, c_is_binary(b18));
            acc.add(18, addition, fp_sub(b18, f.next(18)));
            acc.add(37, doubling, c_is_binary(b37));
            acc.add(37, addition, fp_sub(b37, f.next(37)));
        }
    }
    fp *o = p.out + (size_t)kk * n + j;
    *o = (PART == SF_DBL0 && !AFTER_SPLIT) ? acc.total : fp_add(*o, acc.total);
}

constexpr int SCH_SPLIT_EC_TABLES = 8, SCH_SPLIT_TABLES = 11;
template <int PART>
__global__ __launch_bounds__(FNT, CS_EC_WAVES) void k_schnorr_ec_split(const fp *__restrict__ lde, const fp *__restrict__ aux, const fp *__restrict__ coefs_tx_layout,
                                                                      fp *__restrict__ out, unsigned log_n) {
    const size_t n = (size_t)1 << log_n;
    const size_t j = blockIdx.x * (size_t)FNT + threadIdx.x;
    const unsigned kc = blockIdx.y, kk = 2 * kc;
    const fp *base = lde + (size_t)kk * 56 * n;
    Frame f;
    f.n = n;
    f.cur_p = base + j;
    f.next_p = base + ((j + 1) & (n - 1));
    f.per_p = nullptr;
    f.pcycle = 512;
    SplitAcc<1> acc;
    acc.coefs = as_const(coefs_tx_layout);
    fp *fam = out + (size_t)(PART == PART_DBL0 || PART == PART_DBL1 ? 0 : 3) * 4 * n;
    if (PART == PART_DBL0) fused_doubling(acc, f, 0, (fp)0);
    if (PART == PART_DBL1) fused_doubling(acc, f, 19, (fp)0);
    if (PART == PART_ADD0) fused_addition(acc, f, 0, const6(c_generator), const6(c_generator + 6), (fp)0);
    if (PART == PART_ADD1) {
        acc.begin();
#pragma unroll
        for (int i = 0; i < 18; i++) acc.term(19 + i, fp_sub(f.next(19 + i), f.cur(19 + i)));
#pragma unroll
        for (int q = 0; q < 2; q++) {
            fp *o = fam + ((size_t)q * 4 + kc) * n + j;
            *o = fp_add(*o, acc.result(0, q));
        }
        const fp *ax = aux + (size_t)kk * 19 * n + j;
        const Point pt = {load6(f, 19, false), load6(f, 25, false), load6(f, 31, false)};
        const Point a = ec_add_mixed<CS_EC_CALL>(pt, fp6_load_strided(ax, n), fp6_load_strided(ax + 6 * n, n));
        acc.begin();
#pragma unroll
        for (int i = 0; i < 6; i++) {
            acc.term(19 + i, fp_sub(a.x.c[i], pt.x.c[i]));
            acc.term(25 + i, fp_sub(a.y.c[i], pt.y.c[i]));
            acc.term(31 + i, fp_sub(a.z.c[i], pt.z.c[i]));
        }
        fam = out + (size_t)6 * 4 * n;
    }
    constexpr int NQ = PART == PART_ADD1 ? 2 : 3;
#pragma unroll
    for (int q = 0; q < NQ; q++) {
        fp *o = fam + ((size_t)q * 4 + kc) * n + j;
        const fp v = acc.result(0, q);
        *o = PART == PART_DBL1 ? fp_add(*o, v) : v;
    }
}
__global__ __launch_bounds__(FNT, CS_EC_WAVES) void k_schnorr_final_split(const fp *__restrict__ lde, const fp *__restrict__ coefs_tx_layout, fp *__restrict__ out,
                                                                         unsigned log_n, int coset) {
    const size_t n = (size_t)1 << log_n;
    const size_t j = blockIdx.x * (size_t)FNT + threadIdx.x;
    const unsigned kc = blockIdx.y, kk = coset < 0 ? 2 * kc : (unsigned)coset;
    const fp *base = lde + (size_t)kk * 56 * n;
    Frame f;
    f.n = n;
    f.cur_p = base + j;
    f.next_p = base + ((j + 1) & (n - 1));
    f.per_p = nullptr;
    f.pcycle = 512;
    SplitAcc<1> acc;
    acc.coefs = as_const(coefs_tx_layout);
    fused_final_addition(acc, f, (fp)0);
#pragma unroll
    for (int q = 0; q < 3; q++) {
        if (coset < 0) out[((size_t)q * 4 + kc) * n + j] = acc.result(0, q);
        else out[(size_t)q * n + j] = acc.result(0, q);
    }
}
template <int T>
__global__ __launch_bounds__(256) void k_schnorr_split_finish(AirCombineParams p, const fp *__restrict__ even, const fp *__restrict__ odd,
                                                              const fp *__restrict__ ptab, unsigned g0, unsigned g1, const fp *__restrict__ hi) {
    const size_t n = (size_t)1 << p.log_n;
    const size_t j = blockIdx.x * (size_t)256 + threadIdx.x;
    const unsigned k = blockIdx.y;
    const fp x0 = fp_mul(p.tgrp_shift[k][g0], p.w[(j * p.tgrp_adj[g0]) & (n - 1)]), x1 = fp_mul(p.tgrp_shift[k][g1], p.w[(j * p.tgrp_adj[g1]) & (n - 1)]);
    const fp *per = ptab + (size_t)k * 36 * 512 + (j & 511);
    const fp scalar_mult = per[(size_t)1 * 512], doubling = per[(size_t)2 * 512];
    const fp addition = fp_mul(c_not(doubling), scalar_mult);
    const fp bit37 = p.lde[((size_t)k * 56 + 37) * n + j];
    auto value = [&](int t) { return (k & 1) ? odd[((size_t)(k >> 1) * T + t) * n + j] : even[((size_t)t * 4 + (k >> 1)) * n + j]; };
    const fp dbl = fp_add(value(0), fp_add(fp_mul(value(1), x0), fp_mul(value(2), x1)));
    const fp add = fp_add(value(3), fp_add(fp_mul(value(4), x0), fp_mul(value(5), x1)));
    const fp addbit = fp_add(value(6), fp_mul(value(7), x0));
    fp total = fp_add(fp_mul(doubling, dbl), fp_mul(addition, fp_sub(add, fp_mul(bit37, addbit))));
    if (T > SCH_SPLIT_EC_TABLES) {
        fp fa = value(8), fb0 = value(9), fb1 = value(10);
        if (k & 1) {
            const fp *h = hi + (size_t)(k >> 1) * 3 * n + j;
            fa = fp_sub(fa, fp_dbl(h[0]));
            fb0 = fp_sub(fb0, fp_dbl(h[n]));
            fb1 = fp_sub(fb1, fp_dbl(h[2 * n]));
        }
        const fp final_add = fp_mul(c_not(scalar_mult), per[0]);
        total = fp_add(total, fp_mul(final_add, fp_add(fa, fp_add(fp_mul(fb0, x0), fp_mul(fb1, x1)))));
    }
    p.out[(size_t)k * n + j] = total;
}

struct AirSumView {
    AirSum &a;
    __device__ __forceinline__ fp coef(int, int i) const { return a.coef(i); }
// ... 188 lines not shown
    } else {
        fp den[AIR_MAX_GROUPS], pre[AIR_MAX_GROUPS], run = FP_ONE;
        for (unsigned g = 0; g < p.n_agrp; g++) {
            den[g] = fp_sub(fp_mul(p.agrp_mshift[k][g], p.w[(j * p.agrp_m[g]) & mask]), p.agrp_zc[g]);
            xb[g] = fp_mul(p.agrp_bshift[k][g], p.w[(j * p.agrp_badj[g]) & mask]);
            pre[g] = run;
            run = fp_mul(run, den[g]);
        }
        fp inv = fp_inv(run);
        for (unsigned g = p.n_agrp; g-- > 0;) {
            zi[g] = fp_mul(inv, pre[g]);
            inv = fp_mul(inv, den[g]);
        }
    }
    fp acc = 0;
    if (p.tsum) acc = p.tsum[(size_t)kk * n + j];
    else
        for (unsigned i = 0; i < p.n_constraints; i++)
            acc = fp_add(acc, fp_mul(p.evals[((size_t)kk * p.n_constraints + i) * n + j], fp_add(p.t_alpha[i], fp_mul(p.t_beta[i], xp[p.t_grp[i]]))));
    acc = fp_mul(acc, fp_mul(fp_sub(x, p.w_last), p.zinv_coset[k]));
    for (unsigned g = 0; g < p.n_agrp; g++) {
        Acc128 sa = acc_zero(), sb = acc_zero();
        int cnt = 0;
        for (unsigned a = 0; a < p.n_assertions; a++) {
            if (p.a_grp[a] != g) continue;
            const fp tv = p.lde[((size_t)kk * p.width + p.a_reg[a]) * n + j];
            const fp cv = p.a_seq[a] >= 0 ? p.avals[((size_t)kk * p.n_avals + p.a_seq[a]) * n + j] : p.a_value[a];
            const fp d = fp_sub(tv, cv);
            acc_mad(sa, p.b_alpha[a], d);
            acc_mad(sb, p.b_beta[a], d);
            if (++cnt == 7) { acc_fold(sa); acc_fold(sb); cnt = 0; }
        }
        acc_fold(sa); acc_fold(sb);
        acc = fp_add(acc, fp_mul(fp_add(acc_reduce(sa), fp_mul(xb[g], acc_reduce(sb))), zi[g]));
    }
    *o = acc;
}

}

hipError_t launch_eval_transitions(const CeParams &p, unsigned nk, hipStream_t stream) {
    const size_t n = (size_t)1 << p.log_n;
    hipError_t e = hipMemsetAsync(p.out, 0, (size_t)nk * 115 * n * sizeof(fp), stream);
    if (e != hipSuccess) return e;
    hipLaunchKernelGGL(k_eval_transitions, dim3((unsigned)(n / NT), nk), dim3(NT), 0, stream, p);
    return hipGetLastError();
}
hipError_t launch_eval_frames(const uint64_t *cur, const uint64_t *next, const uint64_t *per, uint64_t *out, unsigned nf, hipStream_t stream) {
    if (nf == 0) return hipSuccess;
    hipLaunchKernelGGL(k_eval_frames, dim3((nf + NT - 1) / NT), dim3(NT), 0, stream, cur, next, per, out, nf);
    return hipGetLastError();
}
hipError_t launch_eval_transitions_merkle(const uint64_t *lde, const uint64_t *ptab, uint64_t *out, unsigned log_n, unsigned k0, unsigned nk,
                                          hipStream_t stream) {
    const size_t n = (size_t)1 << log_n;
    hipError_t e = hipMemsetAsync(out, 0, (size_t)nk * 106 * n * sizeof(fp), stream);
    if (e != hipSuccess) return e;
    hipLaunchKernelGGL(k_eval_transitions_merkle, dim3((unsigned)(n / NT), nk), dim3(NT), 0, stream, lde, ptab, out, log_n, k0);
    return hipGetLastError();
}
hipError_t launch_eval_transitions_schnorr(const uint64_t *lde, const uint64_t *aux, const uint64_t *ptab, uint64_t *out, unsigned log_n, unsigned k0,
                                           unsigned nk, hipStream_t stream) {
    const size_t n = (size_t)1 << log_n;
    hipError_t e = hipMemsetAsync(out, 0, (size_t)nk * 56 * n * sizeof(fp), stream);
    if (e != hipSuccess) return e;
    hipLaunchKernelGGL(k_eval_transitions_schnorr<0>, dim3((unsigned)(n / NT), nk), dim3(NT), 0, stream, lde, aux, ptab, out, log_n, k0);
    hipLaunchKernelGGL(k_eval_transitions_schnorr<1>, dim3((unsigned)(n / NT), nk), dim3(NT), 0, stream, lde, aux, ptab, out, log_n, k0);
    hipLaunchKernelGGL(k_eval_transitions_schnorr<2>, dim3((unsigned)(n / NT), nk), dim3(NT), 0, stream, lde, aux, ptab, out, log_n, k0);
    hipLaunchKernelGGL(k_eval_transitions_schnorr<3>, dim3((unsigned)(n / NT), nk), dim3(NT), 0, stream, lde, aux, ptab, out, log_n, k0);
    return hipGetLastError();
}
hipError_t launch_schnorr_fused(const AirCombineParams &p, const uint64_t *aux, const uint64_t *ptab, unsigned nk, hipStream_t stream) {
    const size_t n = (size_t)1 << p.log_n;
    if (n % FNT) return hipErrorInvalidValue;
    const dim3 grid((unsigned)(n / FNT), nk), block(FNT);
    hipLaunchKernelGGL(k_schnorr_fused<SF_DBL0>, grid, block, 0, stream, p, aux, ptab);
    hipLaunchKernelGGL(k_schnorr_fused<SF_ADD0>, grid, block, 0, stream, p, aux, ptab);
    hipLaunchKernelGGL(k_schnorr_fused<SF_DBL1>, grid, block, 0, stream, p, aux, ptab);
    hipLaunchKernelGGL(k_schnorr_fused<SF_ADD1>, grid, block, 0, stream, p, aux, ptab);
    hipLaunchKernelGGL(k_schnorr_fused<SF_FINAL>, grid, block, 0, stream, p, aux, ptab);
    hipLaunchKernelGGL(k_schnorr_fused<SF_REST>, grid, block, 0, stream, p, aux, ptab);
    return hipGetLastError();
}
hipError_t launch_schnorr_ec_split(const AirCombineParams &p, const uint64_t *aux, const uint64_t *d_coefs_tx_layout, uint64_t *d_even, hipStream_t stream) {
    const size_t n = (size_t)1 << p.log_n;
    if (n % FNT) return hipErrorInvalidValue;
    const dim3 grid((unsigned)(n / FNT), 4), block(FNT);
    hipLaunchKernelGGL(k_schnorr_ec_split<PART_DBL0>, grid, block, 0, stream, p.lde, aux, d_coefs_tx_layout, d_even, p.log_n);
    hipLaunchKernelGGL(k_schnorr_ec_split<PART_DBL1>, grid, block, 0, stream, p.lde, aux, d_coefs_tx_layout, d_even, p.log_n);
    hipLaunchKernelGGL(k_schnorr_ec_split<PART_ADD0>, grid, block, 0, stream, p.lde, aux, d_coefs_tx_layout, d_even, p.log_n);
    hipLaunchKernelGGL(k_schnorr_ec_split<PART_ADD1>, grid, block, 0, stream, p.lde, aux, d_coefs_tx_layout, d_even, p.log_n);
    return hipGetLastError();
}
hipError_t launch_schnorr_final_split(const AirCombineParams &p, const uint64_t *d_coefs_tx_layout, uint64_t *d_out, int coset, hipStream_t stream) {
    const size_t n = (size_t)1 << p.log_n;
    if (n % FNT) return hipErrorInvalidValue;
    hipLaunchKernelGGL(k_schnorr_final_split, dim3((unsigned)(n / FNT), coset < 0 ? 4 : 1), dim3(FNT), 0, stream, p.lde, d_coefs_tx_layout, d_out, p.log_n, coset);
    return hipGetLastError();
}
static bool merkle_rounds_on_matrix_cores(size_t n) {
    static const bool env = [] { const char *e = getenv("CSTARK_ROUNDS_MFMA"); return !e || atoi(e) != 0; }();
    return env && n % 256 == 0;
}
hipError_t launch_schnorr_split_finish(const AirCombineParams &p, const uint64_t *aux, const uint64_t *ptab, const uint64_t *d_even, const uint64_t *d_odd,
                                       unsigned g0, unsigned g1, hipStream_t stream, uint64_t *d_rtab, unsigned round_group, const uint64_t *d_hi) {
    const size_t n = (size_t)1 << p.log_n;
    if (n % FNT) return hipErrorInvalidValue;
    const dim3 grid((unsigned)(n / FNT), 8), block(FNT);
    if (d_hi) {
        hipLaunchKernelGGL(k_schnorr_split_finish<SCH_SPLIT_TABLES>, dim3((unsigned)(n / 256), 8), dim3(256), 0, stream, p, d_even, d_odd, ptab, g0, g1, d_hi);
    } else {
        hipLaunchKernelGGL(k_schnorr_split_finish<SCH_SPLIT_EC_TABLES>, dim3((unsigned)(n / 256), 8), dim3(256), 0, stream, p, d_even, d_odd, ptab, g0, g1, d_hi);
        hipLaunchKernelGGL((k_schnorr_fused<SF_FINAL, true>), grid, block, 0, stream, p, aux, ptab);
    }
    if (d_rtab) {
        hipLaunchKernelGGL((k_merkle_rounds_setup<4, 36, 8>), dim3(2), dim3(64), 0, stream, p.t_alpha, p.t_beta, ptab, d_rtab, 8u);
        if (merkle_rounds_on_matrix_cores(n)) { const hipError_t e = launch_merkle_rounds_mfma(p, ptab, d_rtab, 8, round_group, 1, stream); if (e != hipSuccess) return e; }
        else hipLaunchKernelGGL((k_merkle_rounds<4, 1, 56, 36, 7, 8, true>), grid, block, 0, stream, p, ptab, (const fp *)d_rtab, round_group);
        hipLaunchKernelGGL((k_schnorr_fused<SF_REST, true, true>), grid, block, 0, stream, p, aux, ptab);
    } else {
        hipLaunchKernelGGL((k_schnorr_fused<SF_REST, true>), grid, block, 0, stream, p, aux, ptab);
    }
    return hipGetLastError();
}
hipError_t launch_merkle_fused(const AirCombineParams &p, const uint64_t *ptab, unsigned nk, hipStream_t stream, uint64_t *d_rtab, unsigned round_group) {
    const size_t n = (size_t)1 << p.log_n;
    if (n % FNT) return hipErrorInvalidValue;
    const dim3 grid((unsigned)(n / FNT), nk);
    if (!d_rtab) {
        hipLaunchKernelGGL(k_merkle_fused<false>, grid, dim3(FNT), 0, stream, p, ptab);
        return hipGetLastError();
    }
    if (p.k0 + nk > 8) return hipErrorInvalidValue;
    hipLaunchKernelGGL((k_merkle_rounds_setup<0, 33, 5>), dim3(MR_SECTIONS), dim3(64), 0, stream, p.t_alpha, p.t_beta, ptab, d_rtab, p.k0 + nk);
    if (merkle_rounds_on_matrix_cores(n)) { const hipError_t e = launch_merkle_rounds_mfma(p, ptab, d_rtab, nk, round_group, 0, stream); if (e != hipSuccess) return e; }
    else hipLaunchKernelGGL((k_merkle_rounds<0, 4, 65, 33, 4, 5, false>), grid, dim3(FNT), 0, stream, p, ptab, (const fp *)d_rtab, round_group);
    hipLaunchKernelGGL(k_merkle_fused<true>, grid, dim3(FNT), 0, stream, p, ptab);
    return hipGetLastError();
}
template <class Acc>
__device__ __forceinline__ void rescue_transitions(Acc &acc, const Frame &f) {
    const fp hash_flag = f.pv(0), copy_flag = c_not(hash_flag);
    Frame fr = f;
    fr.per_p = f.per_p - (size_t)(P_ARK - 1) * f.pcycle;
    enforce_round(acc, fr, 0, 0, hash_flag, 0, 0, false);
    for (int i = 0; i < 7; i++) {
        acc.add(i, copy_flag, fp_sub(f.cur(i), f.next(i)));
        acc.add(7 + i, copy_flag, f.next(7 + i));
    }
}
__global__ __launch_bounds__(NT) void k_eval_transitions_rescue(const fp *lde, const fp *ptab, fp *out, unsigned log_n, unsigned k0) {
    const size_t n = (size_t)1 << log_n;
    const size_t j = blockIdx.x * (size_t)NT + threadIdx.x;
    if (j >= n) return;
    const unsigned kk = blockIdx.y;
    const fp *base = lde + (size_t)kk * 14 * n;
    Frame f;
    f.n = n;
    f.cur_p = base + j;
    f.next_p = base + ((j + 1) & (n - 1));
    f.per_p = ptab + (size_t)(k0 + kk) * 29 * 8 + (j & 7);
    f.pcycle = 8;
    AccAll acc{out + (size_t)kk * 14 * n + j, n};
    rescue_transitions(acc, f);
}
template <int AIR, int NC>
__global__ __launch_bounds__(NT) void k_eval_frames_sub(const fp *__restrict__ cur, const fp *__restrict__ next, const fp *__restrict__ per,
                                                        fp *__restrict__ out, unsigned nf) {
    const unsigned j = blockIdx.x * NT + threadIdx.x;
    if (j >= nf) return;
    Frame f;
    f.n = nf;
    f.cur_p = cur + j;
    f.next_p = next + j;
    f.per_p = per + j;
    f.pcycle = nf;
#pragma unroll 1
    for (int i = 0; i < NC; i++) out[(size_t)i * nf + j] = 0;
    AccAll acc{out + j, nf};
    if (AIR == 1) merkle_transitions(acc, f);
    else if (AIR == 3) range_transitions(acc, f);
    else rescue_transitions(acc, f);
}
hipError_t launch_eval_frames_air(int air, const uint64_t *cur, const uint64_t *next, const uint64_t *per, uint64_t *out, unsigned nf, hipStream_t stream) {
    if (nf == 0) return hipSuccess;
    const dim3 grid((nf + NT - 1) / NT), block(NT);
    if (air == 0) hipLaunchKernelGGL(k_eval_frames, grid, block, 0, stream, cur, next, per, out, nf);
    else if (air == 1) hipLaunchKernelGGL((k_eval_frames_sub<1, 106>), grid, block, 0, stream, cur, next, per, out, nf);
    else if (air == 3) hipLaunchKernelGGL((k_eval_frames_sub<3, 2>), grid, block, 0, stream, cur, next, per, out, nf);
    else if (air == 4) hipLaunchKernelGGL((k_eval_frames_sub<4, 14>), grid, block, 0, stream, cur, next, per, out, nf);
    else if (air == 2) {
        hipLaunchKernelGGL(k_eval_frames_schnorr<0>, grid, block, 0, stream, cur, next, per, out, nf);
        hipLaunchKernelGGL(k_eval_frames_schnorr<1>, grid, block, 0, stream, cur, next, per, out, nf);
        hipLaunchKernelGGL(k_eval_frames_schnorr<2>, grid, block, 0, stream, cur, next, per, out, nf);
        hipLaunchKernelGGL(k_eval_frames_schnorr<3>, grid, block, 0, stream, cur, next, per, out, nf);
    } else return hipErrorInvalidValue;
    return hipGetLastError();
}
hipError_t launch_eval_transitions_rescue(const uint64_t *lde, const uint64_t *ptab, uint64_t *out, unsigned log_n, unsigned k0, unsigned nk,
                                          hipStream_t stream) {
    const size_t n = (size_t)1 << log_n;
    hipError_t e = hipMemsetAsync(out, 0, (size_t)nk * 14 * n * sizeof(fp), stream);
    if (e != hipSuccess) return e;
    hipLaunchKernelGGL(k_eval_transitions_rescue, dim3((unsigned)((n + NT - 1) / NT), nk), dim3(NT), 0, stream, lde, ptab, out, log_n, k0);
    return hipGetLastError();
}
hipError_t launch_eval_transitions_range(const uint64_t *lde, uint64_t *out, unsigned log_n, unsigned nk, hipStream_t stream) {
    const size_t n = (size_t)1 << log_n;
    hipLaunchKernelGGL(k_eval_transitions_range, dim3((unsigned)((n + 63) / 64), nk), dim3(64), 0, stream, lde, out, log_n);
    return hipGetLastError();
}
__global__ void k_assert_inverses(fp *__restrict__ tab, const fp *__restrict__ w, AssertShifts sh, uint64_t m, fp zc, unsigned log_n) {
    const size_t n = (size_t)1 << log_n, period = n / m;
    const size_t i = blockIdx.x * (size_t)blockDim.x + threadIdx.x;
    if (i >= period) return;
    const unsigned k = blockIdx.y;
    tab[(size_t)k * period + i] = fp_inv(fp_sub(fp_mul(sh.s[k], w[(i * m) & (n - 1)]), zc));
}
hipError_t launch_assert_inverses(uint64_t *d_tab, const uint64_t *d_w, const uint64_t shift_m[8], unsigned b, uint64_t m, uint64_t zc, unsigned log_n,
                                  hipStream_t stream) {
    const size_t period = ((size_t)1 << log_n) / m;
    AssertShifts sh;
    for (unsigned k = 0; k < 8; k++) sh.s[k] = k < b ? shift_m[k] : 0;
    hipLaunchKernelGGL(k_assert_inverses, dim3((unsigned)((period + 255) / 256), b), dim3(256), 0, stream, d_tab, d_w, sh, m, zc, log_n);
    return hipGetLastError();
}
hipError_t launch_air_combine(const AirCombineParams &p, unsigned nk, hipStream_t stream) {
    const size_t n = (size_t)1 << p.log_n;
    hipLaunchKernelGGL(k_air_combine, dim3((unsigned)((n + 63) / 64), nk), dim3(64), 0, stream, p);
    return hipGetLastError();
}

template <class Fn>
static hipError_t with_sets(unsigned m, Fn fn) {
    if (m == 1) fn(std::integral_constant<int, 1>{});
    else if (m == 2) fn(std::integral_constant<int, 2>{});
    else if (m == 3) fn(std::integral_constant<int, 3>{});
    else return hipErrorInvalidValue;
    return hipGetLastError();
}

hipError_t launch_rounds_setup(const CeParams &p, hipStream_t stream) {
    const unsigned m = p.m ? p.m : 1;
    if (m > 3) return hipErrorInvalidValue;
#ifdef CS_ROUNDS_MFMA
    (void)hipMemsetAsync(p.rtab + RT_MT, 0, MT_BYTES, stream);
    hipLaunchKernelGGL(k_rounds_setup, dim3(RT_SECTIONS + 14, m), dim3(64), 0, stream, p.coef, p.ptab, p.rtab);
#else
    hipLaunchKernelGGL(k_rounds_setup, dim3(RT_SECTIONS, m), dim3(64), 0, stream, p.coef, p.ptab, p.rtab);
#endif
    return hipGetLastError();
}
hipError_t launch_rounds_split(const CeParams &p, uint64_t *d_even, hipStream_t stream) {
    const size_t n = (size_t)1 << p.log_n;
    const dim3 grid((unsigned)(n / FNT), p.nkc ? p.nkc : 4), block(FNT);
    const unsigned m = p.m ? p.m : 1;
    static const bool mfma_env = [] { const char *e = getenv("CSTARK_ROUNDS_MFMA"); return !e || atoi(e) != 0; }();
    if (m <= 3 && mfma_env && n % 512 == 0) return launch_rounds_mfma(p, d_even, stream);
    return with_sets(m, [&](auto M) { hipLaunchKernelGGL(k_rounds_split<M>, grid, block, 0, stream, p, d_even); });
}
hipError_t launch_ec_split(const CeParams &p, int part, uint64_t *d_even_family, uint64_t *d_even_linear, hipStream_t stream) {
    const size_t n = (size_t)1 << p.log_n;
    const dim3 grid((unsigned)(n / FNT), p.nkc ? p.nkc : 4), block(FNT);
    const unsigned m = p.m ? p.m : 1;
    if (part != PART_DBL0 && part != PART_DBL1 && part != PART_ADD0 && part != PART_ADD1) return hipErrorInvalidValue;
    return with_sets(m, [&](auto M) {
        if (part == PART_DBL0) hipLaunchKernelGGL((k_ec_split<PART_DBL0, false, M>), grid, block, 0, stream, p, d_even_family, d_even_linear);
        else if (part == PART_DBL1) hipLaunchKernelGGL((k_ec_split<PART_DBL1, true, M>), grid, block, 0, stream, p, d_even_family, d_even_linear);
        else if (part == PART_ADD0) hipLaunchKernelGGL((k_ec_split<PART_ADD0, false, M>), grid, block, 0, stream, p, d_even_family, d_even_linear);
        else hipLaunchKernelGGL((k_ec_split<PART_ADD1, false, M>), grid, block, 0, stream, p, d_even_family, d_even_linear);
    });
}
hipError_t launch_lin_all(const CeParams &p, uint64_t *d_even_family0, hipStream_t stream) {
    const size_t n = (size_t)1 << p.log_n;
    const dim3 grid((unsigned)(n / FNT), p.nkc ? p.nkc : 4), block(FNT);
    const unsigned m = p.m ? p.m : 1;
    const bool buf = p.log_n <= 22;
    for (unsigned set = 0; set < m; set++) {
        if (buf) hipLaunchKernelGGL(k_lin_all<true>, grid, block, 0, stream, p, d_even_family0, set);
        else hipLaunchKernelGGL(k_lin_all<false>, grid, block, 0, stream, p, d_even_family0, set);
    }
    return hipGetLastError();
}
hipError_t launch_split_finish(const CeParams &p, const uint64_t *d_even, const uint64_t *d_odd, const uint64_t *d_hi, hipStream_t stream, bool merged) {
    const size_t n = (size_t)1 << p.log_n;
    const dim3 grid((unsigned)(n / 256), 8), block(256);
    const unsigned m = p.m ? p.m : 1;
    return with_sets(m, [&](auto M) {
        if (merged) hipLaunchKernelGGL((k_split_finish<M, true>), grid, block, 0, stream, p, d_even, d_odd, d_hi);
        else hipLaunchKernelGGL((k_split_finish<M, false>), grid, block, 0, stream, p, d_even, d_odd, d_hi);
    });
}
hipError_t launch_final_hi_merged(const CeParams &p, const uint64_t *d_odd, const uint64_t *d_direct, uint64_t *d_hi, uint64_t half_m, hipStream_t stream) {
    const size_t n = (size_t)1 << p.log_n;
    const unsigned m = p.m ? p.m : 1;
    const dim3 grid((unsigned)(n / 256), m), block(256);
    if (p.k0 != 0) return hipErrorInvalidValue;
    return with_sets(m, [&](auto M) { hipLaunchKernelGGL(k_final_hi_merged<M>, grid, block, 0, stream, p, d_odd, d_direct, d_hi, half_m); });
}
hipError_t launch_final_hi_merge(const CeParams &p, const uint64_t *d_tco, const uint64_t *d_qco, uint64_t *d_out, const CosetMergeTerm &tm, uint64_t half_m,
                                 hipStream_t stream) {
    const size_t n = (size_t)1 << p.log_n;
    const unsigned m = p.m ? p.m : 1;
    const dim3 grid((unsigned)(n / 256), m), block(256);
    if (tm.r >= n) return hipErrorInvalidValue;
    return with_sets(m, [&](auto M) { hipLaunchKernelGGL(k_final_hi_merge<M>, grid, block, 0, stream, d_tco, d_qco, d_out, n, tm, half_m); });
}
hipError_t launch_split_finish_shard(const CeParams &p, const uint64_t *d_even, const uint64_t *d_odd, const uint64_t *d_hi, const uint64_t *d_bit37_all,
                                     uint64_t *d_out, hipStream_t stream) {
    const size_t n = (size_t)1 << p.log_n;
    if (p.nkc != 1 && p.nkc != 2) return hipErrorInvalidValue;
    hipLaunchKernelGGL(k_split_finish_shard, dim3((unsigned)(n / 256), p.nkc + 4), dim3(256), 0, stream, p, d_even, d_odd, d_hi, d_bit37_all, d_out);
    return hipGetLastError();
}
hipError_t launch_shard_combine(const uint64_t *d_parts, uint64_t *d_out, unsigned log_n, unsigned nkc, hipStream_t stream) {
    const size_t n = (size_t)1 << log_n;
    if (nkc != 1 && nkc != 2) return hipErrorInvalidValue;
    hipLaunchKernelGGL(k_shard_combine, dim3((unsigned)(n / 256), 8), dim3(256), 0, stream, d_parts, d_out, log_n, nkc);
    return hipGetLastError();
}
hipError_t launch_final_split(const CeParams &p, int coset, uint64_t *d_out, hipStream_t stream) {
    const size_t n = (size_t)1 << p.log_n;
    const unsigned even_rows = p.nkc ? p.nkc : 4;
    const dim3 grid((unsigned)(n / FNT), coset < 0 ? even_rows : 1), block(FNT);
    const unsigned m = p.m ? p.m : 1;
    return with_sets(m, [&](auto M) { hipLaunchKernelGGL(k_final_split<M>, grid, block, 0, stream, p, d_out, coset); });
}
hipError_t launch_final_hi(const uint64_t *d_odd, const uint64_t *d_direct, uint64_t *d_hi, uint64_t half_m, unsigned log_n, unsigned rows, unsigned first,
                           unsigned per_set, unsigned tables_per_set, hipStream_t stream) {
    const size_t n = (size_t)1 << log_n;
    if (n % 256 || rows == 0 || per_set == 0 || rows % per_set || first + per_set > tables_per_set) return hipErrorInvalidValue;
    hipLaunchKernelGGL(k_final_hi, dim3((unsigned)(n / 256), rows), dim3(256), 0, stream, d_odd, d_direct, d_hi, half_m, log_n, first, per_set, tables_per_set);
    return hipGetLastError();
}

hipError_t launch_eval_constraints(const CeParams &p, unsigned nk, hipStream_t stream, hipEvent_t *part_events) {
    const size_t n = (size_t)1 << p.log_n;
    const dim3 grid((unsigned)(n / FNT), nk), block(FNT);
    const unsigned m = p.m ? p.m : 1;
    hipError_t e = launch_rounds_setup(p, stream);
    if (e != hipSuccess) return e;
#define CS_PART(PART)                                                                                                                   \
    if (part_events) (void)hipEventRecord(part_events[PART], stream);                                                                   \
    e = with_sets(m, [&](auto M) {                                                                                                      \
        if (PART == PART_ROUNDS && ROUNDS_DYN_LDS)                                                                                      \
            (void)hipFuncSetAttribute((const void *)k_eval_fused<PART, M>, hipFuncAttributeMaxDynamicSharedMemorySize, (int)ROUNDS_LDS); \
        hipLaunchKernelGGL((k_eval_fused<PART, M>), grid, block, PART == PART_ROUNDS ? ROUNDS_DYN_LDS : 0, stream, p);                  \
    });                                                                                                                                 \
    if (e != hipSuccess) return e;
    CS_PART(PART_ROUNDS) CS_PART(PART_DBL0) CS_PART(PART_ADD0) CS_PART(PART_DBL1) CS_PART(PART_ADD1) CS_PART(PART_FINAL)
    CS_PART(PART_LIN_A) CS_PART(PART_LIN_B) CS_PART(PART_LIN_C)
#undef CS_PART
// ... 24 lines not shown
```

certificate-stark_amd/csrc/ctx.h:

```cpp
#pragma once
#include <stdlib.h>
#include <hip/hip_runtime.h>
#include <stdio.h>
#include <deque>
#include <vector>
#include "../../include/cstark.h"
#include "constraints.h"
#include "trace_gen.h"
#include "witness_layout.h"

#include <chrono>
namespace cs {
inline hipError_t stream_wait(hipStream_t st) {
    static const bool block = [] { const char *e = getenv("CSTARK_SYNC_BLOCK"); return e && atoi(e) != 0; }();
    static const long spin_us = [] { const char *e = getenv("CSTARK_SPIN_US"); return e ? atol(e) : 200L; }();
    if (block || spin_us <= 0) return hipStreamSynchronize(st);
    const auto t0 = std::chrono::steady_clock::now();
    hipError_t e;
    for (unsigned it = 0; (e = hipStreamQuery(st)) == hipErrorNotReady; it++) {
#if defined(__x86_64__) || defined(__i386__)
        __builtin_ia32_pause();
#endif
        if ((it & 15) == 15 && std::chrono::duration_cast<std::chrono::microseconds>(std::chrono::steady_clock::now() - t0).count() > spin_us)
            return hipStreamSynchronize(st);
// ... 40 lines not shown

struct NttPlan {
    unsigned log_n;
    uint64_t *w, *winv;
    uint64_t n_inv;
    uint64_t *aux_w = nullptr, *aux_winv = nullptr;
};
struct CosetTable {
    unsigned log_n, log_b;
    uint64_t offset;
    uint64_t *s;
    uint64_t *aux = nullptr;
    size_t aux_words = 0;
};
struct StepTable {
    unsigned log_n, log_b;
    uint64_t offset;
    unsigned log_block;
    unsigned split;
    uint64_t *d;
    uint64_t *w;
};
struct PeriodicTable {
    unsigned depth, log_n, log_b;
    uint64_t *tab;
    uint64_t *coset;
    uint64_t *binv;
    int air = 0;
};
struct AssertInverseTable {
    unsigned log_n, log_b;
    uint64_t m, zc;
    uint64_t *tab;
};
struct AirCombineStatic {
    int air;
    uint32_t n_items, log_n, log_b;
    AirCombineParams p;
    std::vector<uint32_t> t_grp;
    uint64_t *d_static;
};
enum class AirTransitions {
    Materialised,
    MerkleFused,
    SchnorrFused,
};
struct AirStageRequest {
    int air = 0;
    uint32_t n_items = 0;
    uint32_t log_n = 0, log_blowup = 0, k0 = 0, nk = 0;
    const uint64_t *d_lde = nullptr;
    uint64_t *d_out = nullptr;
    AirTransitions source = AirTransitions::Materialised;
    const uint64_t *d_evals = nullptr;
    uint32_t merkle_depth = 0;
    const uint64_t *d_aux_lde = nullptr;
    bool own_extension = false;
    const uint64_t *t_alpha = nullptr, *t_beta = nullptr, *b_alpha = nullptr, *b_beta = nullptr, *assertion_values = nullptr;
    const uint64_t *d_coefs = nullptr, *d_avalues = nullptr;
    const uint64_t *d_avals_lde = nullptr;
    uint32_t n_avals = 0;
};
struct ProveArena;
void prove_arena_free(ProveArena *a);
struct VerifyArena;
void verify_arena_free(VerifyArena *a);

}

struct cstark_ctx {
    int device = 0;
    hipStream_t stream = nullptr;
    bool owns_stream = false;
    hipStream_t side = nullptr, side2 = nullptr;
    hipEvent_t ev_fork = nullptr, ev_join = nullptr, ev_join2 = nullptr, ev_mid = nullptr;
    void *wit_buf = nullptr;
    size_t wit_bytes = 0;
    cs::TxWitnessDev wit{};
    std::deque<cs::NttPlan> plans;
    std::deque<cs::CosetTable> cosets;
    std::deque<cs::StepTable> steps;
    std::deque<cs::PeriodicTable> periodic;
    uint64_t *coef_buf = nullptr;
    void *coef_stage = nullptr;
    hipEvent_t coef_ev = nullptr;
    std::deque<cs::AssertInverseTable> assert_inv;
    std::deque<cs::AirCombineStatic> air_static;
    uint64_t *air_coef_buf = nullptr, *air_coef_stage = nullptr;
    size_t air_coef_words = 0;
    hipEvent_t air_coef_ev = nullptr;
    uint64_t *deep_buf = nullptr, *deep_stage = nullptr;
    size_t deep_words = 0;
    hipEvent_t deep_ev = nullptr;
    std::deque<cs::PeriodicTable> small_periodic;
    void *desc_buf = nullptr;
    hipEvent_t part_ev[cs::CE_NUM_PARTS + 1] = {};
    bool part_timing = false, part_valid = false;
    std::vector<hipEvent_t> lde_ev;
    size_t lde_ev_used = 0;
    uint64_t lde_units = 0;
    uint64_t *tail_buf = nullptr;
    std::vector<uint64_t> schnorr_rx;
    std::vector<uint64_t> schnorr_av_stage;
    std::vector<uint64_t> schnorr_pub;
    std::vector<uint8_t> schnorr_s;
    uint8_t schnorr_seed[32] = {}, schnorr_seed_key[12] = {};
    size_t tail_bytes = 0;
    size_t desc_bytes = 0;
    cs::ProveArena *arena = nullptr;
    cs::VerifyArena *verify = nullptr;
    void *ws = nullptr;
    size_t ws_bytes = 0;
    uint64_t *shard_bit37 = nullptr;
    size_t shard_bit37_words = 0;
    void *rb_dev = nullptr, *rb_host = nullptr;
    size_t rb_dev_bytes = 0, rb_host_bytes = 0;
};
int tx_witness_reserve(cstark_ctx *c, size_t n, size_t d, size_t *sz, size_t *off);
void tx_witness_bind(cstark_ctx *c, size_t n, size_t d, const size_t *off);
int fri_coin_fold_dev(cstark_ctx *c, uint32_t *d_seed, const uint8_t *d_root, uint64_t *d_alpha, uint32_t *d_root_out, const uint64_t *d_evals,
                      uint64_t *d_out, uint32_t log_n, uint32_t log_f, uint64_t domain_offset, uint32_t m);
int hash_rows_slots(cstark_ctx *c, uint32_t hash_fn, const uint64_t *d_lde, uint8_t *d_leaves, uint32_t width, uint32_t log_n, uint32_t log_blowup, uint32_t log_s);
struct cstark_gather_desc {
    const void *src;
    void *out;
    const uint32_t *d_pos, *d_count;
    uint32_t paths, a, log_n, log_b, log_s, count, lvl0;
};
int gather_jobs_launch(cstark_ctx *c, const cstark_gather_desc *jobs, uint32_t n_jobs);
int plan_tables(cstark_ctx *c, unsigned log_n, const uint64_t **w, const uint64_t **winv);

struct cstark_tx_coeffs;
int tx_evaluate_constraints_sets(cstark_ctx *c, const uint64_t *d_lde, const cstark_tx_coeffs *coeffs, uint32_t m, const uint64_t pub_inputs[4],
                                 uint64_t *const *d_outs, uint32_t merkle_depth, uint32_t log_n, uint32_t log_blowup, uint32_t k0, uint32_t nk,
                                 bool input_is_lde, const uint64_t *d_pub = nullptr);
int tx_coef_device_block(cstark_ctx *c, uint64_t **d_coef);
int air_stage(cstark_ctx *c, const cs::AirStageRequest &rq);
int tx_evaluate_constraints_shard(cstark_ctx *c, const uint64_t *d_lde, const uint64_t *d_coeffs, const cstark_tx_coeffs *coeffs, const uint64_t pub_inputs[4],
                                  uint64_t *d_out, uint32_t merkle_depth, uint32_t log_n, uint32_t k0, uint32_t nk);
int tx_shard_combine(cstark_ctx *c, const uint64_t *d_parts, uint64_t *d_out, uint32_t log_n, uint32_t nk);
constexpr uint32_t TX_LATE_COLS = 37;
constexpr uint32_t TX_ROOT_COLS = 58;
constexpr uint32_t TX_COPY_COLS = 65;
constexpr uint32_t TX_STEP_COLS = 27;
int tx_build_trace_split(cstark_ctx *c, uint64_t *d_trace);
int lde_column_range(cstark_ctx *c, const uint64_t *d_coeffs, uint64_t *d_lde, uint32_t width, uint32_t col0, uint32_t ncols, uint32_t log_n,
                     uint32_t log_blowup, uint64_t domain_offset, uint32_t k0, uint32_t nk);
int step_column_range(cstark_ctx *c, uint64_t *d_evals, uint64_t *d_coeffs, uint64_t *d_lde, uint32_t width, uint32_t col0, uint32_t ncols, uint32_t log_n,
                      uint32_t block_len, uint32_t split, uint32_t log_blowup, uint64_t domain_offset, uint32_t k0, uint32_t nk);
int evaluate_ood_frames(cstark_ctx *c, const uint64_t *d_coeffs, uint32_t width, const uint64_t *d_ccoef, uint32_t n_comp, uint32_t log_n,
                        const uint64_t zpts[2], uint64_t zb, uint64_t *out_trace, uint64_t *out_comp);
int ood_frames_dev(cstark_ctx *c, const uint64_t *d_coeffs, uint32_t width, const uint64_t *d_ccoef, uint32_t n_comp, uint32_t log_n, const uint64_t *d_pts,
                   uint64_t *d_out);
int desc_reserve(cstark_ctx *c, size_t bytes);
size_t ood_frames_dev_scratch_bytes(uint32_t width, uint32_t n_comp, uint32_t log_n, uint32_t m);
int ood_frames_dev_ext(cstark_ctx *c, const uint64_t *d_coeffs, uint32_t width, const uint64_t *d_ccoef, uint32_t n_comp, uint32_t log_n, uint32_t m,
                       const uint64_t *d_pts, uint64_t *d_out);
int deep_composition_ext_dev(cstark_ctx *c, const uint64_t *d_trace_lde, const uint64_t *d_comp_lde, uint32_t width, uint32_t n_comp, uint32_t m,
                             const uint64_t *d_coef, const uint64_t *d_ood, uint64_t *d_scal, const uint64_t *d_shifts, uint64_t *d_out, uint32_t log_n,
                             uint32_t log_blowup, uint32_t nk);
int deep_composition_ext_cosets(cstark_ctx *c, const uint64_t *d_trace_lde, const uint64_t *d_comp_lde, uint32_t width, uint32_t n_comp, uint32_t m,
                                const uint64_t *z, const uint64_t *ood_trace, const uint64_t *ood_comp, const uint64_t *alpha, const uint64_t *beta,
                                const uint64_t *delta, const uint64_t *deg_a, const uint64_t *deg_b, uint64_t *d_out, uint32_t log_n, uint32_t log_blowup,
                                uint32_t nk);
```

certificate-stark_amd/csrc/rounds_layout.h:

```cpp
#pragma once
#include "constraints.h"
#include "mds_mfma.cuh"

namespace cs {

struct RoundWindow { int reg, res_a, flag_a, res_b, flag_b; };
#define CS_ROUND_WINDOWS_INIT {{0, 0, 3, 0, -1}, {15, 14, 0, 15, 1}, {29, 28, 0, 29, 1}, {44, 42, 0, 44, 1}, {42, 42, 2, 0, -1}}
#define CS_WINDOW_GROUPS_INIT {{{0, 1, -1}, {-1, -1, -1}}, {{1, 2, 0}, {1, 2, 0}}, {{0, 2, -1}, {0, 2, -1}}, {{2, -1, -1}, {2, -1, -1}}, {{2, -1, -1}, {-1, -1, -1}}}

constexpr int RT_SECTIONS = 5 * 2 * 4;
constexpr int RT_A = 0, RT_UL = RT_SECTIONS * 64, RT_ML = RT_UL + RT_SECTIONS * 14 * 2, RT_MT = RT_ML + 14 * 14 * 2;
constexpr size_t MT_BYTES = (mdsmfma::table_bytes(14) + 15) & ~(size_t)15;
constexpr int RT_G = RT_MT + (int)(MT_BYTES / 8);
constexpr int RT_MF = (RT_G + RT_SECTIONS * 14 + 1) & ~1;

constexpr int MF_TILES_INV = 7, MF_TILES_SEC = 13, MF_KS_INV = 4, MF_KS_SEC = 7;
constexpr int MF_INV_D = RT_MF;
constexpr int MF_SEC_D = MF_INV_D + MF_TILES_INV * 4 * 8;
constexpr int MF_K = MF_SEC_D + MF_TILES_SEC * 4 * 16;
constexpr int RT_SIZE = MF_K + (14 + 2 * MF_TILES_SEC) * 4;
static_assert(RT_SIZE <= CE_RTAB_WORDS, "rtab size");
__host__ __device__ constexpr int mf_tile_base(int w) { return w == 0 ? 0 : w == 1 ? 2 : w == 2 ? 6 : w == 3 ? 10 : w == 4 ? 12 : 13; }
__host__ __device__ constexpr int mf_tile_window(int t) { return t < 2 ? 0 : t < 6 ? 1 : t < 10 ? 2 : t < 12 ? 3 : 4; }
__host__ __device__ constexpr int mf_tile_fs(int w, int local) { return (w == 1 || w == 2) ? local >> 1 : w == 3 ? local : 0; }
__host__ __device__ constexpr int mf_tile_pair(int w, int local) { return (w == 1 || w == 2) ? local & 1 : w == 0 ? local : 0; }

constexpr int MR_SECTIONS = 8, MR_A = 0, MR_UL = MR_SECTIONS * 64, MR_ML = MR_UL + MR_SECTIONS * 14 * 2, MR_G = MR_ML + 196 * 2;
constexpr int MRF_INV_D = MR_G + MR_SECTIONS * 14;
constexpr int MRF_SEC_D = MRF_INV_D + MF_TILES_INV * 32;
constexpr int MRF_K = MRF_SEC_D + 4 * 64;
constexpr int MR_SIZE = MRF_K + (14 + 8) * 4;
static_assert(MR_SIZE <= MERKLE_RTAB_WORDS, "MerkleAir rounds table");

hipError_t launch_merkle_rounds_mfma(const AirCombineParams &p, const uint64_t *ptab, uint64_t *d_rtab, unsigned nk, unsigned round_group, int which,
                                     hipStream_t stream);
hipError_t launch_rounds_mfma(const CeParams &p, uint64_t *d_even, hipStream_t stream);

}
```

Before: 41.69.

## Fold generator-addition constraints into doubling kernel via precomputed quadratic monomial forms

Point addition with the constant generator is expressed as fixed quadratic forms in the six monomials xx, yy, zz, xy, xz, yz. A host-built matrix is folded with the random coefficients on device into lambda vectors. The doubling split kernel already computes those monomials, so it now also produces the generator-addition constraint contributions. This removes the separate ADD0 kernel pass in both the tx and Schnorr paths, saving one full read of the LDE and its extension multiplications. The cost is extra accumulators and register pressure in the doubling kernel, plus a tiny setup kernel.

```diff
diff --git a/certificate-stark_amd/csrc/capi.hip b/certificate-stark_amd/csrc/capi.hip
--- a/certificate-stark_amd/csrc/capi.hip
+++ b/certificate-stark_amd/csrc/capi.hip
@@ -12,6 +12,7 @@
 #include "constraints.h"
 #include "deep.h"
 #include "ext.h"
+#include "generator_fold.h"
 #include "hostfield.h"
 #include "ntt.h"
 #include "trace_gen.h"
@@ -359,6 +360,24 @@
     return CSTARK_OK;
 }
 
+int generator_fold_table(cstark_ctx *c, const uint64_t **d_j) {
+    static_assert(cs::hostg::GF_COMPONENTS == cs::CE_GFOLD_COMPONENTS && cs::hostg::GF_LAMBDA_WORDS == cs::CE_GFOLD_WORDS &&
+                  cs::hostg::GF_OUTPUTS * cs::hostg::GF_COMPONENTS == cs::CE_GFOLD_J_WORDS, "generator fold layout");
+    if (!c->gfold_j) {
+        std::vector<uint64_t> j(cs::CE_GFOLD_J_WORDS);
+        cs::hostg::generator_fold_matrix(j.data());
+        DevGuard keep;
+        uint64_t *d = nullptr;
+        HIP_TRY(keep.alloc(&d, j.size() * 8));
+        HIP_TRY(hipMemcpyAsync(d, j.data(), j.size() * 8, hipMemcpyHostToDevice, c->stream));
+        HIP_TRY(hipStreamSynchronize(c->stream));
+        keep.release();
+        c->gfold_j = d;
+    }
+    *d_j = c->gfold_j;
+    return CSTARK_OK;
+}
+
 int ce_params(cstark_ctx *c, const uint64_t *d_lde, uint64_t *d_out, uint32_t merkle_depth, uint32_t log_n, uint32_t log_blowup, uint32_t k0,
               uint32_t nk, cs::CeParams *p) {
     if (!c || !d_lde || !d_out) return fail(CSTARK_ERR_INVALID_ARG, "constraint evaluation: null argument");
@@ -378,6 +397,7 @@
     for (int g = 0; g < 5; g++) p->adj_mod_n[g] = (uint32_t)(cs::host::tx_group_adjustment(g, n, ce) & (n - 1));
     p->badj_mod_n = (uint32_t)(cs::host::tx_boundary_adjustment(n, ce) & (n - 1));
     p->log_n = log_n; p->log_b = log_blowup; p->k0 = k0;
+    RC_TRY(generator_fold_table(c, &p->gfold_j));
     return CSTARK_OK;
 }
 
@@ -468,6 +488,7 @@
     if (c->wit_buf) (void)hipFree(c->wit_buf);
     if (c->ws) (void)hipFree(c->ws);
     if (c->coef_buf) (void)hipFree(c->coef_buf);
+    if (c->gfold_j) (void)hipFree(c->gfold_j);
     if (c->coef_stage) (void)hipHostFree(c->coef_stage);
     if (c->coef_ev) (void)hipEventDestroy(c->coef_ev);
     for (NttPlan &p : c->plans) { (void)hipFree(p.w); (void)hipFree(p.winv); (void)hipFree(p.aux_w); (void)hipFree(p.aux_winv); }
@@ -1099,9 +1120,8 @@
     HIP_TRY(cs::launch_rounds_split(p, even, stream));
     if (pev) HIP_TRY(hipEventRecord(pev[1], stream));
     uint64_t *fam_dbl = even + (size_t)cs::CE_SPLIT_FAM0 * 4 * n, *fam_add = fam_dbl + 12 * n, *fam_addbit = fam_add + 8 * n;
-    HIP_TRY(cs::launch_ec_split(p, 1, fam_dbl, nullptr, stream));
+    HIP_TRY(cs::launch_ec_split(p, 1, fam_dbl, fam_add, stream));
     if (pev) HIP_TRY(hipEventRecord(pev[2], stream));
-    HIP_TRY(cs::launch_ec_split(p, 2, fam_add, nullptr, stream));
     if (pev) HIP_TRY(hipEventRecord(pev[3], stream));
     HIP_TRY(cs::launch_ec_split(p, 3, fam_dbl, nullptr, stream));
     if (pev) HIP_TRY(hipEventRecord(pev[4], stream));
@@ -1575,7 +1595,9 @@
     const size_t n = st.n, region = (size_t)T * 4 * n, hcol = (size_t)3 * n;
     SplitWs w;
     RC_TRY(split_ws_unmerged(c, region, hcol, &w));
-    HIP_TRY(cs::launch_schnorr_ec_split(p, rq.d_aux_lde, d_txl, w.even, c->stream));
+    const uint64_t *d_gfold_j;
+    RC_TRY(generator_fold_table(c, &d_gfold_j));
+    HIP_TRY(cs::launch_schnorr_ec_split(p, rq.d_aux_lde, d_txl, w.even, d_gfold_j, d_rtab + cs::MERKLE_RTAB_LAMBDA, c->stream));
     if (final5) HIP_TRY(cs::launch_schnorr_final_split(p, d_txl, w.even + (size_t)cs::SCHNORR_SPLIT_EC_TABLES * 4 * n, -1, c->stream));
     RC_TRY(inverse_columns(st, w.even, w.sa, w.sb, 4 * T));
     RC_TRY(even_to_odd(st, w.sb, w.sa, T));
diff --git a/certificate-stark_amd/csrc/constraints.h b/certificate-stark_amd/csrc/constraints.h
--- a/certificate-stark_amd/csrc/constraints.h
+++ b/certificate-stark_amd/csrc/constraints.h
@@ -16,6 +16,7 @@
 constexpr int CE_COEF_WORDS = 115 * 2 + 8;
 constexpr int CE_MAX_SETS = 3;
 constexpr int CE_COSET_CONSTS = 10;
+constexpr int CE_GFOLD_COMPONENTS = 36, CE_GFOLD_WORDS = 3 * CE_GFOLD_COMPONENTS, CE_GFOLD_J_WORDS = 18 * CE_GFOLD_COMPONENTS;
 
 struct CeParams {
     const uint64_t *lde;
@@ -25,6 +26,7 @@
     const uint64_t *coef;
     const uint64_t *binv;
     uint64_t *rtab;
+    const uint64_t *gfold_j;
     uint64_t *out;
     uint64_t *out_ext[CE_MAX_SETS - 1];
     uint32_t m;
@@ -63,11 +65,13 @@
 hipError_t launch_eval_transitions_schnorr(const uint64_t *lde, const uint64_t *aux, const uint64_t *ptab, uint64_t *out, unsigned log_n, unsigned k0,
                                            unsigned nk, hipStream_t stream);
 constexpr int MERKLE_RTAB_WORDS = 2048;
+constexpr int MERKLE_RTAB_LAMBDA = MERKLE_RTAB_WORDS - CE_GFOLD_WORDS;
 hipError_t launch_merkle_fused(const AirCombineParams &p, const uint64_t *ptab, unsigned nk, hipStream_t stream, uint64_t *d_rtab = nullptr,
                                unsigned round_group = 0);
 hipError_t launch_schnorr_fused(const AirCombineParams &p, const uint64_t *aux, const uint64_t *ptab, unsigned nk, hipStream_t stream);
 constexpr int SCHNORR_SPLIT_EC_TABLES = 8, SCHNORR_SPLIT_TABLES = 11;
-hipError_t launch_schnorr_ec_split(const AirCombineParams &p, const uint64_t *aux, const uint64_t *d_coefs_tx_layout, uint64_t *d_even, hipStream_t stream);
+hipError_t launch_schnorr_ec_split(const AirCombineParams &p, const uint64_t *aux, const uint64_t *d_coefs_tx_layout, uint64_t *d_even, const uint64_t *d_gfold_j,
+                                   uint64_t *d_lambda, hipStream_t stream);
 hipError_t launch_schnorr_split_finish(const AirCombineParams &p, const uint64_t *aux, const uint64_t *ptab, const uint64_t *d_even, const uint64_t *d_odd,
                                        unsigned g0, unsigned g1, hipStream_t stream, uint64_t *d_rtab = nullptr, unsigned round_group = 0,
                                        const uint64_t *d_hi = nullptr);
diff --git a/certificate-stark_amd/csrc/constraints.hip b/certificate-stark_amd/csrc/constraints.hip
--- a/certificate-stark_amd/csrc/constraints.hip
+++ b/certificate-stark_amd/csrc/constraints.hip
@@ -438,9 +438,20 @@
 constexpr size_t ROUNDS_DYN_LDS = 0;
 #endif
 
-__global__ void k_rounds_setup(const fp *__restrict__ coef, const fp *__restrict__ ptab, fp *__restrict__ rtab) {
+__device__ __forceinline__ fp generator_fold_entry(const fp *__restrict__ coef, const fp *__restrict__ gfold_j, int e) {
+    const int q = e / CE_GFOLD_COMPONENTS, t = e % CE_GFOLD_COMPONENTS;
+    const int first = q == 2 ? 6 : 0, last = q == 1 ? 6 : 18;
+    fp s = 0;
+    for (int i = first; i < last; i++) s = fp_add(s, fp_mul(coef[(q ? 115 : 0) + i], gfold_j[i * CE_GFOLD_COMPONENTS + t]));
+    return s;
+}
+__global__ void k_rounds_setup(const fp *__restrict__ coef, const fp *__restrict__ ptab, fp *__restrict__ rtab, const fp *__restrict__ gfold_j) {
     coef += (size_t)blockIdx.y * CE_COEF_WORDS;
     rtab += (size_t)blockIdx.y * CE_RTAB_WORDS;
+    if (blockIdx.x == gridDim.x - 1) {
+        for (int e = threadIdx.x; e < CE_GFOLD_WORDS; e += blockDim.x) rtab[RT_LAM + e] = generator_fold_entry(coef, gfold_j, e);
+        return;
+    }
     if (blockIdx.x >= RT_SECTIONS) {
         if (threadIdx.x < 16) mdsmfma::build_table_entry((uint8_t *)(rtab + RT_MT), c_inv_mds, 14, blockIdx.x - RT_SECTIONS, threadIdx.x);
         return;
@@ -929,6 +940,112 @@
         return acc_reduce(a);
     }
 };
+template <int M>
+struct MonoAcc {
+    const CS_CONST fp *lam;
+    int stride;
+    Acc128 s[M][3];
+    int cnt;
+    __device__ __forceinline__ void begin() {
+        cnt = 0;
+#pragma unroll
+        for (int c = 0; c < M; c++) s[c][0] = s[c][1] = s[c][2] = acc_zero();
+    }
+    __device__ __forceinline__ void feed(int m, const Fp6 &v) {
+#pragma unroll
+        for (int k = 0; k < 6; k++) {
+            const bool fold = ++cnt == 7;
+#pragma unroll
+            for (int c = 0; c < M; c++)
+#pragma unroll
+                for (int q = 0; q < 3; q++) {
+                    acc_mad(s[c][q], lam[c * stride + q * CE_GFOLD_COMPONENTS + 6 * m + k], v.c[k]);
+                    if (fold) acc_fold(s[c][q]);
+                }
+            if (fold) cnt = 0;
+        }
+    }
+    __device__ __forceinline__ fp result(int c, int q) {
+        acc_fold(s[c][q]);
+        return acc_reduce(s[c][q]);
+    }
+};
+template <bool CALL>
+__device__ __forceinline__ Point ec_double_from_monomials(const Fp6 &xx, const Fp6 &yy, const Fp6 &zz, const Fp6 &xy, const Fp6 &xz, const Fp6 &yz) {
+#define mul6 MUL6_SEL<CALL>
+    const Fp6 b3 = const6(c_b3);
+    Fp6 t0 = xx, t1 = yy, t2 = zz;
+    Fp6 t3 = fp6_dbl(xy);
+    Fp6 z3 = fp6_dbl(xz);
+    Fp6 y3 = fp6_add(z3, mul6(b3, t2));
+    Fp6 x3 = fp6_sub(t1, y3);
+    y3 = fp6_add(t1, y3);
+    y3 = mul6(x3, y3);
+    x3 = mul6(t3, x3);
+    z3 = mul6(b3, z3);
+    t3 = fp6_add(fp6_sub(t0, t2), z3);
+    t0 = fp6_add(fp6_add(fp6_dbl(t0), t0), t2);
+    y3 = fp6_add(y3, mul6(t0, t3));
+    t2 = fp6_dbl(yz);
+    x3 = fp6_sub(x3, mul6(t2, t3));
+    z3 = fp6_dbl(fp6_dbl(mul6(t2, t1)));
+    return {x3, y3, z3};
+#undef mul6
+}
+template <int M>
+__device__ __forceinline__ void split_doubling_with_generator(SplitAcc<M> &acc, MonoAcc<M> &qa, const Frame &f, fp (&dbl)[M][3], fp (&add)[M][3]) {
+    fp nx[M][3], cu[M][3];
+    acc.begin();
+#pragma unroll
+    for (int i = 0; i < 18; i++) acc.term(i, f.next(i));
+#pragma unroll
+    for (int c = 0; c < M; c++)
+#pragma unroll
+        for (int q = 0; q < 3; q++) nx[c][q] = acc.result(c, q);
+    const Point p = {load6(f, 0, false), load6(f, 6, false), load6(f, 12, false)};
+    acc.begin();
+#pragma unroll
+    for (int i = 0; i < 6; i++) {
+        acc.term(i, p.x.c[i]);
+        acc.term(6 + i, p.y.c[i]);
+        acc.term(12 + i, p.z.c[i]);
+    }
+#pragma unroll
+    for (int c = 0; c < M; c++)
+#pragma unroll
+        for (int q = 0; q < 3; q++) cu[c][q] = acc.result(c, q);
+    qa.begin();
+    const Fp6 xx = MUL6_SEL<CS_EC_CALL>(p.x, p.x);
+    qa.feed(0, xx);
+    const Fp6 yy = MUL6_SEL<CS_EC_CALL>(p.y, p.y);
+    qa.feed(1, yy);
+    const Fp6 zz = MUL6_SEL<CS_EC_CALL>(p.z, p.z);
+    qa.feed(2, zz);
+    const Fp6 xy = MUL6_SEL<CS_EC_CALL>(p.x, p.y);
+    qa.feed(3, xy);
+    const Fp6 xz = MUL6_SEL<CS_EC_CALL>(p.x, p.z);
+    qa.feed(4, xz);
+    const Fp6 yz = MUL6_SEL<CS_EC_CALL>(p.y, p.z);
+    qa.feed(5, yz);
+    const fp bit = f.cur(18);
+#pragma unroll
+    for (int c = 0; c < M; c++)
+#pragma unroll
+        for (int q = 0; q < 3; q++) add[c][q] = fp_sub(fp_sub(nx[c][q], cu[c][q]), fp_mul(bit, fp_sub(qa.result(c, q), cu[c][q])));
+    const Point d = ec_double_from_monomials<CS_EC_CALL>(xx, yy, zz, xy, xz, yz);
+    acc.begin();
+#pragma unroll
+    for (int i = 0; i < 6; i++) {
+        acc.term(i, d.x.c[i]);
+        acc.term(6 + i, d.y.c[i]);
+        acc.term(12 + i, d.z.c[i]);
+    }
+#pragma unroll
+    for (int c = 0; c < M; c++)
+#pragma unroll
+        for (int q = 0; q < 3; q++) dbl[c][q] = fp_sub(nx[c][q], acc.result(c, q));
+}
+
 template <int PART, bool ACCUMULATE, int M>
 #ifndef CS_EC_WAVES
 #define CS_EC_WAVES 2
@@ -941,9 +1058,23 @@
     SplitAcc<M> acc;
     acc.coefs = as_const(p.coef);
     constexpr size_t SET = (size_t)SPLIT_TABLES * 4;
-    if (PART == PART_DBL0) fused_doubling(acc, f, 0, (fp)0);
+    if constexpr (PART == PART_DBL0) {
+        MonoAcc<M> qa;
+        qa.lam = as_const((const fp *)(p.rtab + RT_LAM));
+        qa.stride = CE_RTAB_WORDS;
+        fp dbl[M][3], add[M][3];
+        split_doubling_with_generator(acc, qa, f, dbl, add);
+        const fp xd1 = split_lift(p, 2 * kc, j);
+#pragma unroll
+        for (int c = 0; c < M; c++) {
+#pragma unroll
+            for (int q = 0; q < 3; q++) out[(c * SET + (size_t)q * 4 + kc) * n + j] = dbl[c][q];
+            out_linear[(c * SET + kc) * n + j] = add[c][0];
+            out_linear[(c * SET + 4 + kc) * n + j] = fp_add(add[c][1], fp_mul(xd1, add[c][2]));
+        }
+        return;
+    }
     if (PART == PART_DBL1) fused_doubling(acc, f, 19, (fp)0);
-    if (PART == PART_ADD0) fused_addition(acc, f, 0, const6(c_generator), const6(c_generator + 6), (fp)0);
     if (PART == PART_ADD1) {
         acc.begin();
 #pragma unroll
@@ -965,15 +1096,13 @@
             acc.term(31 + i, fp_sub(a.z.c[i], pt.z.c[i]));
         }
     }
-    constexpr int NQ = (PART == PART_ADD1 || PART == PART_ADD0) ? 2 : 3;
-    const fp xd1 = PART == PART_ADD0 ? split_lift(p, 2 * kc, j) : 0;
+    constexpr int NQ = PART == PART_ADD1 ? 2 : 3;
 #pragma unroll
     for (int c = 0; c < M; c++)
 #pragma unroll
         for (int q = 0; q < NQ; q++) {
             fp *o = out + (c * SET + (size_t)q * 4 + kc) * n + j;
-            fp v = acc.result(c, q);
-            if (PART == PART_ADD0 && q == 1) v = fp_add(v, fp_mul(xd1, acc.result(c, 2)));
+            const fp v = acc.result(c, q);
             *o = ACCUMULATE ? fp_add(*o, v) : v;
         }
 }
@@ -1781,9 +1910,12 @@
 }
 
 constexpr int SCH_SPLIT_EC_TABLES = 8, SCH_SPLIT_TABLES = 11;
+__global__ void k_generator_fold(const fp *__restrict__ coefs_tx_layout, const fp *__restrict__ gfold_j, fp *__restrict__ lam) {
+    for (int e = threadIdx.x; e < CE_GFOLD_WORDS; e += blockDim.x) lam[e] = generator_fold_entry(coefs_tx_layout, gfold_j, e);
+}
 template <int PART>
 __global__ __launch_bounds__(FNT, CS_EC_WAVES) void k_schnorr_ec_split(const fp *__restrict__ lde, const fp *__restrict__ aux, const fp *__restrict__ coefs_tx_layout,
-                                                                      fp *__restrict__ out, unsigned log_n) {
+                                                                      fp *__restrict__ out, unsigned log_n, const fp *__restrict__ lam) {
     const size_t n = (size_t)1 << log_n;
     const size_t j = blockIdx.x * (size_t)FNT + threadIdx.x;
     const unsigned kc = blockIdx.y, kk = 2 * kc;
@@ -1797,9 +1929,20 @@
     SplitAcc<1> acc;
     acc.coefs = as_const(coefs_tx_layout);
     fp *fam = out + (size_t)(PART == PART_DBL0 || PART == PART_DBL1 ? 0 : 3) * 4 * n;
-    if (PART == PART_DBL0) fused_doubling(acc, f, 0, (fp)0);
+    if constexpr (PART == PART_DBL0) {
+        MonoAcc<1> qa;
+        qa.lam = as_const(lam);
+        qa.stride = 0;
+        fp dbl[1][3], add[1][3];
+        split_doubling_with_generator(acc, qa, f, dbl, add);
+#pragma unroll
+        for (int q = 0; q < 3; q++) {
+            fam[((size_t)q * 4 + kc) * n + j] = dbl[0][q];
+            fam[((size_t)(3 + q) * 4 + kc) * n + j] = add[0][q];
+        }
+        return;
+    }
     if (PART == PART_DBL1) fused_doubling(acc, f, 19, (fp)0);
-    if (PART == PART_ADD0) fused_addition(acc, f, 0, const6(c_generator), const6(c_generator + 6), (fp)0);
     if (PART == PART_ADD1) {
         acc.begin();
 #pragma unroll
@@ -2154,14 +2297,15 @@
     hipLaunchKernelGGL(k_schnorr_fused<SF_REST>, grid, block, 0, stream, p, aux, ptab);
     return hipGetLastError();
 }
-hipError_t launch_schnorr_ec_split(const AirCombineParams &p, const uint64_t *aux, const uint64_t *d_coefs_tx_layout, uint64_t *d_even, hipStream_t stream) {
-    const size_t n = (size_t)1 << p.log_n;
-    if (n % FNT) return hipErrorInvalidValue;
+hipError_t launch_schnorr_ec_split(const AirCombineParams &p, const uint64_t *aux, const uint64_t *d_coefs_tx_layout, uint64_t *d_even, const uint64_t *d_gfold_j,
+                                   uint64_t *d_lambda, hipStream_t stream) {
+    const size_t n = (size_t)1 << p.log_n;
+    if (n % FNT || !d_gfold_j || !d_lambda) return hipErrorInvalidValue;
     const dim3 grid((unsigned)(n / FNT), 4), block(FNT);
-    hipLaunchKernelGGL(k_schnorr_ec_split<PART_DBL0>, grid, block, 0, stream, p.lde, aux, d_coefs_tx_layout, d_even, p.log_n);
-    hipLaunchKernelGGL(k_schnorr_ec_split<PART_DBL1>, grid, block, 0, stream, p.lde, aux, d_coefs_tx_layout, d_even, p.log_n);
-    hipLaunchKernelGGL(k_schnorr_ec_split<PART_ADD0>, grid, block, 0, stream, p.lde, aux, d_coefs_tx_layout, d_even, p.log_n);
-    hipLaunchKernelGGL(k_schnorr_ec_split<PART_ADD1>, grid, block, 0, stream, p.lde, aux, d_coefs_tx_layout, d_even, p.log_n);
+    hipLaunchKernelGGL(k_generator_fold, dim3(1), dim3(128), 0, stream, d_coefs_tx_layout, d_gfold_j, d_lambda);
+    hipLaunchKernelGGL(k_schnorr_ec_split<PART_DBL0>, grid, block, 0, stream, p.lde, aux, d_coefs_tx_layout, d_even, p.log_n, (const fp *)d_lambda);
+    hipLaunchKernelGGL(k_schnorr_ec_split<PART_DBL1>, grid, block, 0, stream, p.lde, aux, d_coefs_tx_layout, d_even, p.log_n, (const fp *)d_lambda);
+    hipLaunchKernelGGL(k_schnorr_ec_split<PART_ADD1>, grid, block, 0, stream, p.lde, aux, d_coefs_tx_layout, d_even, p.log_n, (const fp *)d_lambda);
     return hipGetLastError();
 }
 hipError_t launch_schnorr_final_split(const AirCombineParams &p, const uint64_t *d_coefs_tx_layout, uint64_t *d_out, int coset, hipStream_t stream) {
@@ -2314,12 +2458,12 @@
 
 hipError_t launch_rounds_setup(const CeParams &p, hipStream_t stream) {
     const unsigned m = p.m ? p.m : 1;
-    if (m > 3) return hipErrorInvalidValue;
+    if (m > 3 || !p.gfold_j) return hipErrorInvalidValue;
 #ifdef CS_ROUNDS_MFMA
     (void)hipMemsetAsync(p.rtab + RT_MT, 0, MT_BYTES, stream);
-    hipLaunchKernelGGL(k_rounds_setup, dim3(RT_SECTIONS + 14, m), dim3(64), 0, stream, p.coef, p.ptab, p.rtab);
+    hipLaunchKernelGGL(k_rounds_setup, dim3(RT_SECTIONS + 14 + 1, m), dim3(64), 0, stream, p.coef, p.ptab, p.rtab, p.gfold_j);
 #else
-    hipLaunchKernelGGL(k_rounds_setup, dim3(RT_SECTIONS, m), dim3(64), 0, stream, p.coef, p.ptab, p.rtab);
+    hipLaunchKernelGGL(k_rounds_setup, dim3(RT_SECTIONS + 1, m), dim3(64), 0, stream, p.coef, p.ptab, p.rtab, p.gfold_j);
 #endif
     return hipGetLastError();
 }
@@ -2335,11 +2479,11 @@
     const size_t n = (size_t)1 << p.log_n;
     const dim3 grid((unsigned)(n / FNT), p.nkc ? p.nkc : 4), block(FNT);
     const unsigned m = p.m ? p.m : 1;
-    if (part != PART_DBL0 && part != PART_DBL1 && part != PART_ADD0 && part != PART_ADD1) return hipErrorInvalidValue;
+    if (part != PART_DBL0 && part != PART_DBL1 && part != PART_ADD1) return hipErrorInvalidValue;
+    if (part != PART_DBL1 && !d_even_linear) return hipErrorInvalidValue;
     return with_sets(m, [&](auto M) {
         if (part == PART_DBL0) hipLaunchKernelGGL((k_ec_split<PART_DBL0, false, M>), grid, block, 0, stream, p, d_even_family, d_even_linear);
         else if (part == PART_DBL1) hipLaunchKernelGGL((k_ec_split<PART_DBL1, true, M>), grid, block, 0, stream, p, d_even_family, d_even_linear);
-        else if (part == PART_ADD0) hipLaunchKernelGGL((k_ec_split<PART_ADD0, false, M>), grid, block, 0, stream, p, d_even_family, d_even_linear);
         else hipLaunchKernelGGL((k_ec_split<PART_ADD1, false, M>), grid, block, 0, stream, p, d_even_family, d_even_linear);
     });
 }
diff --git a/certificate-stark_amd/csrc/ctx.h b/certificate-stark_amd/csrc/ctx.h
--- a/certificate-stark_amd/csrc/ctx.h
+++ b/certificate-stark_amd/csrc/ctx.h
@@ -146,6 +146,7 @@
     std::deque<cs::StepTable> steps;
     std::deque<cs::PeriodicTable> periodic;
     uint64_t *coef_buf = nullptr;
+    uint64_t *gfold_j = nullptr;
     void *coef_stage = nullptr;
     hipEvent_t coef_ev = nullptr;
     std::deque<cs::AssertInverseTable> assert_inv;
diff --git a/certificate-stark_amd/csrc/generator_fold.h b/certificate-stark_amd/csrc/generator_fold.h
--- /dev/null
+++ b/certificate-stark_amd/csrc/generator_fold.h
@@ -0,0 +1,78 @@
+#pragma once
+#include "hostgadgets.h"
+
+namespace cs { namespace hostg {
+
+constexpr int GF_OUTPUTS = 18, GF_MONOS = 6, GF_COMPONENTS = 36;
+constexpr int GF_FUNCTIONALS = 3;
+constexpr int GF_LAMBDA_WORDS = GF_FUNCTIONALS * GF_COMPONENTS;
+
+struct LinForm { F6 c[3]; };
+struct QuadForm { F6 m[GF_MONOS]; };
+
+inline F6 zero6() { return F6{}; }
+inline F6 one6() { F6 r{}; r.c[0].a = ONE; return r; }
+inline LinForm lin_add(const LinForm &x, const LinForm &y) { return {{add6(x.c[0], y.c[0]), add6(x.c[1], y.c[1]), add6(x.c[2], y.c[2])}}; }
+inline LinForm lin_sub(const LinForm &x, const LinForm &y) { return {{sub6(x.c[0], y.c[0]), sub6(x.c[1], y.c[1]), sub6(x.c[2], y.c[2])}}; }
+inline LinForm lin_scale(const LinForm &x, const F6 &k) { return {{mul6(x.c[0], k), mul6(x.c[1], k), mul6(x.c[2], k)}}; }
+inline QuadForm lin_mul(const LinForm &x, const LinForm &y) {
+    QuadForm q;
+    for (int v = 0; v < 3; v++) q.m[v] = mul6(x.c[v], y.c[v]);
+    q.m[3] = add6(mul6(x.c[0], y.c[1]), mul6(x.c[1], y.c[0]));
+    q.m[4] = add6(mul6(x.c[0], y.c[2]), mul6(x.c[2], y.c[0]));
+    q.m[5] = add6(mul6(x.c[1], y.c[2]), mul6(x.c[2], y.c[1]));
+    return q;
+}
+inline QuadForm quad_add(const QuadForm &x, const QuadForm &y) { QuadForm q; for (int m = 0; m < GF_MONOS; m++) q.m[m] = add6(x.m[m], y.m[m]); return q; }
+inline QuadForm quad_sub(const QuadForm &x, const QuadForm &y) { QuadForm q; for (int m = 0; m < GF_MONOS; m++) q.m[m] = sub6(x.m[m], y.m[m]); return q; }
+
+inline void generator_addition_forms(const F6 &qx, const F6 &qy, QuadForm out[3]) {
+    const F6 b3 = load6(CS_B3_MONT);
+    const LinForm X = {{one6(), zero6(), zero6()}}, Y = {{zero6(), one6(), zero6()}}, Z = {{zero6(), zero6(), one6()}};
+    LinForm t0 = lin_scale(X, qx), t1 = lin_scale(Y, qy);
+    LinForm t3 = lin_sub(lin_scale(lin_add(X, Y), add6(qx, qy)), lin_add(t0, t1));
+    LinForm t4 = lin_add(lin_scale(Z, qx), X), t5 = lin_add(lin_scale(Z, qy), Y);
+    LinForm z3 = lin_add(lin_scale(Z, b3), t4), x3 = lin_sub(t1, z3);
+    z3 = lin_add(t1, z3);
+    QuadForm y3 = lin_mul(x3, z3);
+    t1 = lin_add(lin_add(lin_add(t0, t0), t0), Z);
+    t4 = lin_add(lin_scale(t4, b3), lin_sub(t0, Z));
+    out[1] = quad_add(y3, lin_mul(t1, t4));
+    out[0] = quad_sub(lin_mul(t3, x3), lin_mul(t5, t4));
+    out[2] = quad_add(lin_mul(t5, z3), lin_mul(t3, t1));
+}
+
+inline void generator_fold_monomials(const Pt &p, fp mono[GF_COMPONENTS]) {
+    store6(mono, mul6(p.x, p.x));
+    store6(mono + 6, mul6(p.y, p.y));
+    store6(mono + 12, mul6(p.z, p.z));
+    store6(mono + 18, mul6(p.x, p.y));
+    store6(mono + 24, mul6(p.x, p.z));
+    store6(mono + 30, mul6(p.y, p.z));
+}
+
+inline void generator_fold_matrix(fp J[GF_OUTPUTS * GF_COMPONENTS]) {
+    QuadForm k[3];
+    generator_addition_forms(load6(CS_GENERATOR_MONT), load6(CS_GENERATOR_MONT + 6), k);
+    for (int coord = 0; coord < 3; coord++)
+        for (int m = 0; m < GF_MONOS; m++)
+            for (int c = 0; c < 6; c++) {
+                fp e[6] = {0, 0, 0, 0, 0, 0}, col[6];
+                e[c] = ONE;
+                store6(col, mul6(k[coord].m[m], load6(e)));
+                for (int r = 0; r < 6; r++) J[(6 * coord + r) * GF_COMPONENTS + 6 * m + c] = col[r];
+            }
+}
+
+constexpr int gf_first(int f) { return f == 2 ? 6 : 0; }
+constexpr int gf_last(int f) { return f == 1 ? 6 : GF_OUTPUTS; }
+inline void generator_fold_lambda(const fp *J, const fp *alpha, const fp *beta, fp lambda[GF_LAMBDA_WORDS]) {
+    for (int f = 0; f < GF_FUNCTIONALS; f++)
+        for (int e = 0; e < GF_COMPONENTS; e++) {
+            fp s = 0;
+            for (int i = gf_first(f); i < gf_last(f); i++) s = add(s, mul(f == 0 ? alpha[i] : beta[i], J[i * GF_COMPONENTS + e]));
+            lambda[f * GF_COMPONENTS + e] = s;
+        }
+}
+
+}}
diff --git a/certificate-stark_amd/csrc/rounds_layout.h b/certificate-stark_amd/csrc/rounds_layout.h
--- a/certificate-stark_amd/csrc/rounds_layout.h
+++ b/certificate-stark_amd/csrc/rounds_layout.h
@@ -19,7 +19,8 @@
 constexpr int MF_SEC_D = MF_INV_D + MF_TILES_INV * 4 * 8;
 constexpr int MF_K = MF_SEC_D + MF_TILES_SEC * 4 * 16;
 constexpr int RT_SIZE = MF_K + (14 + 2 * MF_TILES_SEC) * 4;
-static_assert(RT_SIZE <= CE_RTAB_WORDS, "rtab size");
+constexpr int RT_LAM = RT_SIZE;
+static_assert(RT_LAM + CE_GFOLD_WORDS <= CE_RTAB_WORDS, "rtab size");
 __host__ __device__ constexpr int mf_tile_base(int w) { return w == 0 ? 0 : w == 1 ? 2 : w == 2 ? 6 : w == 3 ? 10 : w == 4 ? 12 : 13; }
 __host__ __device__ constexpr int mf_tile_window(int t) { return t < 2 ? 0 : t < 6 ? 1 : t < 10 ? 2 : t < 12 ? 3 : 4; }
 __host__ __device__ constexpr int mf_tile_fs(int w, int local) { return (w == 1 || w == 2) ? local >> 1 : w == 3 ? local : 0; }
@@ -30,7 +31,7 @@
 constexpr int MRF_SEC_D = MRF_INV_D + MF_TILES_INV * 32;
 constexpr int MRF_K = MRF_SEC_D + 4 * 64;
 constexpr int MR_SIZE = MRF_K + (14 + 8) * 4;
-static_assert(MR_SIZE <= MERKLE_RTAB_WORDS, "MerkleAir rounds table");
+static_assert(MR_SIZE <= MERKLE_RTAB_LAMBDA, "MerkleAir rounds table");
 
 hipError_t launch_merkle_rounds_mfma(const AirCombineParams &p, const uint64_t *ptab, uint64_t *d_rtab, unsigned nk, unsigned round_group, int which,
                                      hipStream_t stream);
```

Result: faster. 42.83 (median of 6 runs) (+2.7%).
